# oss0430/SRFRD

Hardware: NVIDIA B200
Metric: training seqs/sec; full-catalogue top-10 users/sec (higher is better)
Workload: dtype bf16

## Files before the change

include/srfrd_b200.h:

```cpp
#ifndef SRFRD_B200_H
#define SRFRD_B200_H

#include <stddef.h>
#include <stdint.h>

#ifdef __cplusplus
extern "C" {
#endif

#define SRFRD_ABI_VERSION 9
#if defined(__GNUC__)
#define SRFRD_API __attribute__((visibility("default")))
#else
#define SRFRD_API
#endif

SRFRD_API const char* srfrd_last_error(void);
SRFRD_API int srfrd_abi_version(void);
SRFRD_API int srfrd_device_check(void);

SRFRD_API int srfrd_embed_ln_fwd(const float* item_table, int64_t n_rows, int D, const float* pos_table,
                       const float* aux_table, int64_t n_aux, int F, int mode, const int64_t* seq,
                       const int64_t* aux_ids, int64_t B, int L, float item_scale, const float* ln_w,
                       const float* ln_b, float eps, void* x0_bf16, float* x0_f32, void* q_bf16, float* stats,
                       int ldx, float drop_p, uint64_t drop_seed, uint32_t drop_stream, const float* drop_step,
                       void* stream);

SRFRD_API int srfrd_srfu_labels(const int64_t* fake_ids, int64_t B, int L, int kind, int64_t* labels, void* stream);

SRFRD_API int srfrd_embed_bwd(const void* dx0_bf16, int ldx, const int64_t* seq, const int64_t* aux_ids, int64_t B, int L,
                    int D, int F, int mode, float item_scale, float* d_item, float* d_aux, void* stream);

SRFRD_API int srfrd_layernorm_fwd(const void* x_bf16, int ldx, const float* w, const float* b, float eps, void* y_bf16,
                        float* y_f32, int ldy, float* stats, int64_t T, int H, int64_t row_stride,
                        int64_t row_offset, void* stream);
SRFRD_API int srfrd_layernorm_bwd(const void* dy_bf16, const float* dy_f32, int lddy, const void* x_bf16, int ldx,
                        const float* stats, const float* w, const void* add_bf16, int ldadd,
                        const int64_t* row_ids, void* dx_bf16, int lddx, float* dw, float* db, int64_t T, int H,
                        void* stream);

typedef struct {
  const float* bias;
  const void* residual;
  const void* gate;
  const int64_t* row_ids;
  void* out_bf16;
  float* out_f32;
  int ldr, ldg, ldc;
  int relu;
  float drop_p;
  uint32_t drop_stream;
  uint64_t drop_seed;
  const float* drop_step;
  void* ln_out_bf16;
  const float* ln_w;
  const float* ln_b;
  float* ln_stats;
  int ld_ln;
  float ln_eps;
} srfrd_gemm_epilogue_t;

SRFRD_API int srfrd_gemm_tn(const void* A_bf16, int lda, const void* B_bf16, int ldb, int M, int N, int K,
                  const srfrd_gemm_epilogue_t* ep, void* stream);
SRFRD_API int srfrd_gemm_tn_plan(int M, int N, int K, int has_aux, int bf16_out, int fused_ln, int* out);
SRFRD_API int srfrd_gemm_debug_read(long long* host_dst);
SRFRD_API int srfrd_attn_debug_read(long long* host_dst);

SRFRD_API int srfrd_gemm_wgrad(const void* dY_bf16, int lda, const void* X_bf16, int ldb, int64_t T, int Mo, int No,
                     float* dW, int ldw, float* dbias, void* stream);
SRFRD_API int srfrd_gemm_ref(const void* A, int lda, const void* B, int ldb, float* C, int ldc, int M, int N, int K,
                   int a_mn_major, int b_mn_major, void* stream);

SRFRD_API int srfrd_colsum(const void* X_bf16, int64_t M, int N, int64_t ld, float* out, void* stream);
SRFRD_API int srfrd_add_segments(float* in, int64_t n, int seg_in, int seg_out, float* out, void* stream);

SRFRD_API int srfrd_dropout_apply(const void* x_bf16, int ldx, void* out_bf16, int ldo, int64_t M, int N, float drop_p,
                        uint64_t seed, uint32_t stream_id, const float* drop_step, void* stream);

typedef struct {
  const float* src; int src_ld;
  void* dst; int dst_ld;
  void* dst_t; int dst_t_ld;
  int rows, cols;
  int dst_is_f32;
} srfrd_cast_desc_t;
SRFRD_API int srfrd_cast_weights(const srfrd_cast_desc_t* descs_dev, int n, void* stream);
SRFRD_API int srfrd_f32_to_bf16_split(const float* src, int64_t src_ld, const int64_t* row_index, void* hi, void* lo,
                            int64_t rows, int cols, int dst_ld, void* stream);

SRFRD_API int srfrd_attention_fwd(const void* q, int ldq, const void* k, const void* v, int ldkv, void* o, int ldo,
                        float* stats, int64_t B, int L, int H, int heads, float drop_p, uint64_t seed, uint32_t stream_id,
                        const float* drop_step, void* stream);
SRFRD_API int srfrd_attention_bwd(const void* dout, int lddo, const void* q, int ldq, const void* k, const void* v, int ldkv,
                        const void* o, int ldo, float* stats, void* dq, int lddq, void* dk, void* dv, int lddkv, int64_t B,
                        int L, int H, int heads, float drop_p, uint64_t seed, uint32_t stream_id, const float* drop_step,
                        void* stream);

SRFRD_API int srfrd_score_fwd(const float* h, int ldh, const float* item_table, const float* fake_table, const int64_t* pos,
                    const int64_t* neg, const int64_t* prs, const int64_t* nrs, int64_t T, int D, int F, float* zp,
                    float* zn, void* stream);
SRFRD_API int srfrd_score_bwd(const float* h, int ldh, const float* item_table, const float* fake_table, const int64_t* pos,
                    const int64_t* neg, const int64_t* prs, const int64_t* nrs, const float* dzp, const float* dzn,
                    int64_t T, int D, int F, float* dh, int lddh, float* d_item, float* d_fake, void* stream);
SRFRD_API int srfrd_score_loss_fused(const float* h, int ldh, const float* item_table, const float* fake_table,
                           const int64_t* pos, const int64_t* neg, const int64_t* prs, const int64_t* nrs,
                           const float* w_pos, const float* w_neg, const float* norm, int64_t T, int D, int F,
                           float* zp, float* zn, float* loss_acc, float* dh, int lddh, float* d_item, float* d_fake,
                           void* stream);
SRFRD_API int srfrd_weight_sums(const int64_t* pos, const float* w_pos, const float* w_neg, int64_t T, float* out2,
                      void* stream);
SRFRD_API int srfrd_loss_finalize(float* acc2, const float* norm2, float* loss, void* stream);

SRFRD_API int srfrd_adam_tick(float* state3, float beta1, float beta2, void* stream);
SRFRD_API int srfrd_adam_step(float* p, float* g, float* m, float* v, int64_t n, float lr, float beta1, float beta2, float eps,
                    const float* state3, int zero_grad, void* stream);

SRFRD_API int srfrd_adam_step_fused(float* p, float* g, float* m, float* v, int64_t n, float lr, float beta1, float beta2,
                          float eps, float* state8, int zero_grad, float* acc2, const float* norm2, float* loss,
                          void* stream, const int64_t* l2_seg, int l2_n_seg, const float* l2_coef, const float* l2_reg);

SRFRD_API int srfrd_param_l2_plan(const int64_t* seg_host, int n_seg, int64_t* n_chunks);
SRFRD_API int srfrd_param_l2(const float* p, const int64_t* seg, int n_seg, int64_t n_chunks, float l2, float* coef,
                   float* reg, double* ws, void* stream);

#define SRFRD_TOPK_KMAX 64
SRFRD_API int srfrd_catalogue_topk_plan(int64_t U, int64_t n_rows, int64_t row_lo, int D, int n_split, int* chunks_out,
                                        int k);
SRFRD_API int srfrd_catalogue_topk_kmax(int D, int n_split, int* kmax_out);
SRFRD_API int srfrd_catalogue_topk(const void* feats_bf16, int64_t U, int64_t u_pad, int n_split, const void* table_bf16,
                         int64_t n_rows, int64_t row_lo, int64_t id_base, int D, int ld_feats, int ld_table,
                         int chunks, float* part_scores, int* part_ids, float* packed_out, void* stream, int k);
SRFRD_API int srfrd_merge_topk(const float* scores, const int* ids, int64_t U, int nlists, int k, float* out_scores,
                     int64_t* out_ids, void* stream);
SRFRD_API int srfrd_merge_topk_packed(const float* packed, int64_t U, int nlists, int k, float* out_scores,
                            int64_t* out_ids, void* stream);
SRFRD_API int srfrd_catalogue_rank(const void* feats_bf16, int64_t U, int64_t u_pad, int n_split,
                                   const void* table_bf16, int64_t n_rows, int64_t row_lo, int64_t id_base,
                                   int D, int ld_feats, int ld_table,
                                   const void* target_rows_bf16, int ld_target, const int64_t* target_ids,
                                   float* target_scores, int* rank_out, void* stream);

SRFRD_API int srfrd_sample_batch(const int64_t* offsets, const int* items, const int8_t* labels, const float* p_fake,
                       const int* eligible, int n_eligible, int itemnum, int B, int L, int policy, uint64_t seed,
                       const float* step, int64_t* users, int64_t* seq, int64_t* rsq, int64_t* pos, int64_t* prs,
                       int64_t* neg, int64_t* nrs, float* w_pos, void* stream);

SRFRD_API int srfrd_sample_candidates(const int64_t* offsets, const int* items, const int* users0, const int* target,
                            int64_t U, int itemnum, int C, uint64_t seed, int64_t* cand, void* stream);
SRFRD_API int srfrd_candidate_rank(const float* feats, int ldf, const float* item_table, int64_t n_rows, int D,
                         const int64_t* cand, int64_t U, int C, const float* fake_table, int F,
                         const int64_t* user_label, float* logits, int ldl, int* rank, int* err_flag, void* stream);
SRFRD_API int srfrd_add_user_term(float* logits, int ldl, int64_t U, int I, const float* feats_tail, int ldf,
                        const float* fake_table, const int64_t* label, int F, void* stream);

typedef struct {
  int* rows;
  int* cnt;
  int* seq_first;
  int* tok_row;
  int* row_tok;
  int64_t* row_ids;
  int* row_info;
  int* tile_row0;
  int* last_row;
  int64_t cap;
} srfrd_pack_t;
SRFRD_API int srfrd_pack_plan(const int64_t* seq, const int64_t* keep, int64_t B, int L, const srfrd_pack_t* pk, void* stream);
SRFRD_API int srfrd_set_row_limit(const int* rows_dev);
SRFRD_API int srfrd_embed_ln_fwd_packed(const float* item_table, int64_t n_rows, int D, const float* pos_table,
                              const float* aux_table, int64_t n_aux, int F, int mode, const int64_t* seq,
                              const int64_t* aux_ids, int64_t B, int L, float item_scale, const float* ln_w,
                              const float* ln_b, float eps, void* x0_bf16, void* q_bf16, float* stats, int ldx,
                              float drop_p, uint64_t drop_seed, uint32_t drop_stream, const float* drop_step,
                              const int* row_tok, const int* rows_dev, int64_t cap_rows, void* stream);
SRFRD_API int srfrd_layernorm_fwd_rows(const void* x_bf16, int ldx, const float* w, const float* b, float eps, float* y_f32,
                             int ldy, const int* row_index, int64_t n, int H, void* stream);
SRFRD_API int srfrd_attention_packed_supported(int L, int H, int heads);
SRFRD_API int srfrd_attention_packed_oproj_supported(int L, int H, int heads);
SRFRD_API int srfrd_attention_fwd_packed(const void* q, int ldq, const void* k, const void* v, int ldkv, void* o, int ldo,
                               const srfrd_pack_t* pk, int L, int H, int heads, float drop_p, uint64_t seed,
                               uint32_t stream_id, const float* drop_step, void* stream, const void* wo, int ldw,
                               const float* bo, const void* res, int ldres, const float* ln_w, const float* ln_b,
                               float ln_eps, float* ln_stats, void* r, int ldr, void* y, int ldy);
SRFRD_API int srfrd_attention_bwd_packed(const void* dout, int lddo, const void* q, int ldq, const void* k, const void* v,
                               int ldkv, void* dq, int lddq, void* dk, void* dv, int lddkv, const srfrd_pack_t* pk,
                               int L, int H, int heads, float drop_p, uint64_t seed, uint32_t stream_id,
                               const float* drop_step, void* stream, const void* dr, int lddr, const void* woT, int ldw);
SRFRD_API int srfrd_score_loss_fused_packed(const float* h, int ldh, const float* item_table, const float* fake_table,
                                  const int64_t* pos, const int64_t* neg, const int64_t* prs, const int64_t* nrs,
                                  const float* w_pos, const float* w_neg, const float* norm, int D, int F,
                                  float* loss_acc, float* dh, int lddh, float* d_item, float* d_fake,
                                  const int* row_tok, const int* rows_dev, int64_t cap_rows, void* stream);
SRFRD_API int srfrd_embed_bwd_packed(const void* dx0_bf16, int ldx, const int64_t* seq, const int64_t* aux_ids,
                           const int* row_tok, const int* rows_dev, int64_t cap_rows, int L, int D, int F, int mode,
                           float item_scale, float* d_item, float* d_aux, float* d_pos, void* stream);

typedef struct {
  const float* bias1; const float* bias2;
  const void* gate; int ldg;
  int relu1;
  float drop1_p, drop2_p; uint32_t drop1_stream, drop2_stream; uint64_t drop_seed; const float* drop_step;
  const void* residual; int ldr;
  int residual_is_a;
  const int64_t* row_ids;
  void* mid_out; int ldm;
  void* out; int ldc;
  void* ln_out; int ld_ln; const float* ln_w; const float* ln_b; float* ln_stats; float ln_eps;
} srfrd_mlp2_t;
SRFRD_API int srfrd_mlp2_tn(const void* A_bf16, int lda, const void* W1_bf16, int ldw1, const void* W2_bf16, int ldw2, int M, int N,
                  const srfrd_mlp2_t* ep, void* stream);

SRFRD_API int srfrd_attention_live_items(const int* tok_row, int64_t B, int L, int heads, int* q_lo, int* items, int* n_live,
                               void* stream);
SRFRD_API int srfrd_set_attention_live(const int* q_lo, const int* items, const int* n_live, const int* tok_row);

typedef struct {
  const void* src; int ld_s;
  void* dst; int ld_d;
  int W;
  int mode;
} srfrd_repack_part_t;
SRFRD_API int srfrd_unpack_rows(const srfrd_repack_part_t* parts, int n_parts, const srfrd_pack_t* pk, int64_t B, int L,
                      void* stream);
SRFRD_API int srfrd_pack_rows(const srfrd_repack_part_t* parts, int n_parts, const srfrd_pack_t* pk, int64_t B, int L,
                    void* stream);

SRFRD_API int srfrd_dp_adam_step(float* const* grad_ptrs_dev, float* const* param_ptrs_dev, uint32_t* const* signal_ptrs_dev,
                       int rank, int world, int64_t n, float* m, float* v, float lr, float beta1, float beta2, float eps,
                       float* state8, const float* norm2, uint32_t* local4, void* stream, const int64_t* l2_seg,
                       int l2_n_seg, const float* l2_coef, const float* l2_reg);

#ifdef __cplusplus
}
#endif
#endif
```

srfrd_b200/_lib.py:

```python
from __future__ import annotations

import ctypes as C
import os

_HERE = os.path.dirname(os.path.abspath(__file__))
LIB_PATH = os.environ.get("SRFRD_B200_LIB") or os.path.join(_HERE, "lib", "libsrfrd_b200.so")

vp, i32, i64, f32, u32, u64 = C.c_void_p, C.c_int, C.c_int64, C.c_float, C.c_uint32, C.c_uint64


class GemmEpilogue(C.Structure):
    _fields_ = [("bias", vp), ("residual", vp), ("gate", vp), ("row_ids", vp), ("out_bf16", vp), ("out_f32", vp),
                ("ldr", i32), ("ldg", i32), ("ldc", i32), ("relu", i32), ("drop_p", f32), ("drop_stream", u32),
                ("drop_seed", u64), ("drop_step", vp),
                ("ln_out_bf16", vp), ("ln_w", vp), ("ln_b", vp), ("ln_stats", vp), ("ld_ln", i32), ("ln_eps", f32)]


class CastDesc(C.Structure):
    _fields_ = [("src", vp), ("src_ld", i32), ("dst", vp), ("dst_ld", i32), ("dst_t", vp), ("dst_t_ld", i32),
                ("rows", i32), ("cols", i32), ("dst_is_f32", i32)]


class Mlp2Epilogue(C.Structure):
    _fields_ = [("bias1", vp), ("bias2", vp), ("gate", vp), ("ldg", i32), ("relu1", i32), ("drop1_p", f32), ("drop2_p", f32),
                ("drop1_stream", u32), ("drop2_stream", u32), ("drop_seed", u64), ("drop_step", vp), ("residual", vp), ("ldr", i32),
                ("residual_is_a", i32), ("row_ids", vp), ("mid_out", vp), ("ldm", i32), ("out", vp), ("ldc", i32),
                ("ln_out", vp), ("ld_ln", i32), ("ln_w", vp), ("ln_b", vp), ("ln_stats", vp), ("ln_eps", f32)]


class PackDesc(C.Structure):
    _fields_ = [("rows", vp), ("cnt", vp), ("seq_first", vp), ("tok_row", vp), ("row_tok", vp), ("row_ids", vp),
                ("row_info", vp), ("tile_row0", vp), ("last_row", vp), ("cap", i64)]


class RepackPart(C.Structure):
    _fields_ = [("src", vp), ("ld_s", i32), ("dst", vp), ("ld_d", i32), ("W", i32), ("mode", i32)]


SIGNATURES = {
    "srfrd_abi_version": [],
    "srfrd_device_check": [],
    "srfrd_embed_ln_fwd": [vp, i64, i32, vp, vp, i64, i32, i32, vp, vp, i64, i32, f32, vp, vp, f32, vp, vp, vp, vp, i32,
                           f32, u64, u32, vp, vp],
    "srfrd_srfu_labels": [vp, i64, i32, i32, vp, vp],
    "srfrd_embed_bwd": [vp, i32, vp, vp, i64, i32, i32, i32, i32, f32, vp, vp, vp],
    "srfrd_layernorm_fwd": [vp, i32, vp, vp, f32, vp, vp, i32, vp, i64, i32, i64, i64, vp],
    "srfrd_layernorm_bwd": [vp, vp, i32, vp, i32, vp, vp, vp, i32, vp, vp, i32, vp, vp, i64, i32, vp],
    "srfrd_gemm_tn": [vp, i32, vp, i32, i32, i32, i32, C.POINTER(GemmEpilogue), vp],
    "srfrd_mlp2_tn": [vp, i32, vp, i32, vp, i32, i32, i32, C.POINTER(Mlp2Epilogue), vp],
    "srfrd_gemm_tn_plan": [i32, i32, i32, i32, i32, i32, vp],
    "srfrd_gemm_debug_read": [vp],
    "srfrd_attn_debug_read": [vp],
    "srfrd_gemm_wgrad": [vp, i32, vp, i32, i64, i32, i32, vp, i32, vp, vp],
    "srfrd_gemm_ref": [vp, i32, vp, i32, vp, i32, i32, i32, i32, i32, i32, vp],
    "srfrd_colsum": [vp, i64, i32, i64, vp, vp],
    "srfrd_add_segments": [vp, i64, i32, i32, vp, vp],
    "srfrd_dropout_apply": [vp, i32, vp, i32, i64, i32, f32, u64, u32, vp, vp],
    "srfrd_cast_weights": [vp, i32, vp],
    "srfrd_f32_to_bf16_split": [vp, i64, vp, vp, vp, i64, i32, i32, vp],
    "srfrd_attention_fwd": [vp, i32, vp, vp, i32, vp, i32, vp, i64, i32, i32, i32, f32, u64, u32, vp, vp],
    "srfrd_attention_bwd": [vp, i32, vp, i32, vp, vp, i32, vp, i32, vp, vp, i32, vp, vp, i32, i64, i32, i32, i32, f32, u64,
                            u32, vp, vp],
    "srfrd_score_fwd": [vp, i32, vp, vp, vp, vp, vp, vp, i64, i32, i32, vp, vp, vp],
    "srfrd_score_bwd": [vp, i32, vp, vp, vp, vp, vp, vp, vp, vp, i64, i32, i32, vp, i32, vp, vp, vp],
    "srfrd_score_loss_fused": [vp, i32, vp, vp, vp, vp, vp, vp, vp, vp, vp, i64, i32, i32, vp, vp, vp, vp, i32, vp, vp, vp],
    "srfrd_weight_sums": [vp, vp, vp, i64, vp, vp],
    "srfrd_loss_finalize": [vp, vp, vp, vp],
    "srfrd_adam_tick": [vp, f32, f32, vp],
    "srfrd_adam_step": [vp, vp, vp, vp, i64, f32, f32, f32, f32, vp, i32, vp],
    "srfrd_adam_step_fused": [vp, vp, vp, vp, i64, f32, f32, f32, f32, vp, i32, vp, vp, vp, vp, vp, i32, vp, vp],
    "srfrd_param_l2_plan": [C.POINTER(i64), i32, C.POINTER(i64)],
    "srfrd_param_l2": [vp, vp, i32, i64, f32, vp, vp, vp, vp],
    "srfrd_catalogue_topk_plan": [i64, i64, i64, i32, i32, C.POINTER(i32), i32],
    "srfrd_catalogue_topk_kmax": [i32, i32, C.POINTER(i32)],
    "srfrd_catalogue_topk": [vp, i64, i64, i32, vp, i64, i64, i64, i32, i32, i32, i32, vp, vp, vp, vp, i32],
    "srfrd_merge_topk_packed": [vp, i64, i32, i32, vp, vp, vp],
    "srfrd_catalogue_rank": [vp, i64, i64, i32, vp, i64, i64, i64, i32, i32, i32, vp, i32, vp, vp, vp, vp],
    "srfrd_attention_live_items": [vp, i64, i32, i32, vp, vp, vp, vp],
    "srfrd_set_attention_live": [vp, vp, vp, vp],
    "srfrd_merge_topk": [vp, vp, i64, i32, i32, vp, vp, vp],
    "srfrd_unpack_rows": [C.POINTER(RepackPart), i32, C.POINTER(PackDesc), i64, i32, vp],
    "srfrd_pack_rows": [C.POINTER(RepackPart), i32, C.POINTER(PackDesc), i64, i32, vp],
    "srfrd_dp_adam_step": [vp, vp, vp, i32, i32, i64, vp, vp, f32, f32, f32, f32, vp, vp, vp, vp, vp, i32, vp, vp],
    "srfrd_pack_plan": [vp, vp, i64, i32, C.POINTER(PackDesc), vp],
    "srfrd_set_row_limit": [vp],
    "srfrd_embed_ln_fwd_packed": [vp, i64, i32, vp, vp, i64, i32, i32, vp, vp, i64, i32, f32, vp, vp, f32, vp, vp, vp, i32,
                                  f32, u64, u32, vp, vp, vp, i64, vp],
    "srfrd_layernorm_fwd_rows": [vp, i32, vp, vp, f32, vp, i32, vp, i64, i32, vp],
    "srfrd_attention_packed_supported": [i32, i32, i32],
    "srfrd_attention_packed_oproj_supported": [i32, i32, i32],
    "srfrd_attention_fwd_packed": [vp, i32, vp, vp, i32, vp, i32, C.POINTER(PackDesc), i32, i32, i32, f32, u64, u32, vp, vp,
                                   vp, i32, vp, vp, i32, vp, vp, f32, vp, vp, i32, vp, i32],
    "srfrd_attention_bwd_packed": [vp, i32, vp, i32, vp, vp, i32, vp, i32, vp, vp, i32, C.POINTER(PackDesc), i32, i32, i32,
                                   f32, u64, u32, vp, vp, vp, i32, vp, i32],
    "srfrd_score_loss_fused_packed": [vp, i32, vp, vp, vp, vp, vp, vp, vp, vp, vp, i32, i32, vp, vp, i32, vp, vp, vp, vp,
                                      i64, vp],
    "srfrd_embed_bwd_packed": [vp, i32, vp, vp, vp, vp, i64, i32, i32, i32, i32, f32, vp, vp, vp, vp],
    "srfrd_sample_candidates": [vp, vp, vp, vp, i64, i32, i32, u64, vp, vp],
    "srfrd_candidate_rank": [vp, i32, vp, i64, i32, vp, i64, i32, vp, i32, vp, vp, i32, vp, vp, vp],
    "srfrd_add_user_term": [vp, i32, i64, i32, vp, i32, vp, vp, i32, vp],
    "srfrd_sample_batch": [vp, vp, vp, vp, vp, i32, i32, i32, i32, i32, u64, vp, vp, vp, vp, vp, vp, vp, vp, vp, vp],
}

_lib = None
_device_ok = False
launch_count = 0


def load() -> C.CDLL:
    global _lib
    if _lib is not None:
        return _lib
    if not os.path.exists(LIB_PATH):
        raise RuntimeError(
            f"srfrd_b200: {LIB_PATH} is not built. Run `make -C srfrd_b200/csrc` (needs nvcc, sm_100a). "
            "There is no CPU fallback.")
    lib = C.CDLL(LIB_PATH)
    lib.srfrd_last_error.restype = C.c_char_p
    lib.srfrd_last_error.argtypes = []
    for name, argtypes in SIGNATURES.items():
        fn = getattr(lib, name)
        fn.argtypes = argtypes
        fn.restype = C.c_int
    if lib.srfrd_abi_version() != 9:
        raise RuntimeError("srfrd_b200: ABI version mismatch between _lib.py and the built library")
    _lib = lib
    return lib


def require_device() -> None:
    global _device_ok
    if _device_ok:
        return
    lib = load()
    if lib.srfrd_device_check() != 0:
        raise RuntimeError("srfrd_b200: " + lib.srfrd_last_error().decode())
    _device_ok = True


_profile = None


def set_profile(records) -> None:
    global _profile
    _profile = records


def call(name: str, *args) -> None:
    global launch_count
    lib = _lib or load()
    if _profile is not None:
        import torch
        e0, e1 = torch.cuda.Event(enable_timing=True), torch.cuda.Event(enable_timing=True)
        e0.record()
        rc = getattr(lib, name)(*args)
        e1.record()
        _profile.append((name, args, e0, e1))
    else:
        rc = getattr(lib, name)(*args)
    if rc != 0:
        raise RuntimeError(f"{name}: {lib.srfrd_last_error().decode()}")
    launch_count += 1
```

srfrd_b200/csrc/ffn.cu:

```cuda
#include <stdlib.h>

#include "common.cuh"
#include "srfrd_b200.h"

namespace srfrd {

static constexpr int MLP_THREADS = 160;
static constexpr int MT = 128;
static constexpr int MBLK = MT * 64 * 2;

struct MlpParams {
  int M, N, kb;
  int K, kbk;
  int single;
  int relu2; const bf16* gate2; int ldg2;
  const int* rows_dev;
  const float *bias1, *bias2;
  const bf16* gate; int ldg;
  int relu1;
  uint64_t drop_seed; const float* drop_step;
  uint32_t thresh1, thresh2, stream1, stream2; float scale1, scale2;
  const bf16* residual; int ldr;
  int residual_is_a;
  const int64_t* row_ids;
  const float *ln_w, *ln_b; float* ln_stats; float ln_eps; int has_ln;
};

__device__ __forceinline__ uint32_t swz_chunk(int r, int j) { return (uint32_t)(r * 128 + ((j ^ (r & 7)) << 4)); }
__device__ __forceinline__ void mlp_bar_sync() { asm volatile("bar.sync 1, 128;" ::: "memory"); }
__device__ __forceinline__ void mlp_tma_store(const CUtensorMap* tmap, const void* smem_src, int c0, int c1) {
  asm volatile("cp.async.bulk.tensor.2d.global.shared::cta.bulk_group [%0, {%2, %3}], [%1];" ::"l"(tmap),
               "r"(smem_u32(smem_src)), "r"(c0), "r"(c1)
               : "memory");
}
__device__ __forceinline__ void unpack8_bf16(const uint4& u, float* f) {
  const uint32_t w[4] = {u.x, u.y, u.z, u.w};
#pragma unroll
  for (int i = 0; i < 4; ++i) { f[2 * i] = __uint_as_float(w[i] << 16); f[2 * i + 1] = __uint_as_float(w[i] & 0xffff0000u); }
}

__global__ void __launch_bounds__(MLP_THREADS, 2)
mlp2_kernel(const __grid_constant__ CUtensorMap tmA, const __grid_constant__ CUtensorMap tmW1,
            const __grid_constant__ CUtensorMap tmW2, const __grid_constant__ CUtensorMap tmMid,
            const __grid_constant__ CUtensorMap tmOut, const __grid_constant__ CUtensorMap tmLn, MlpParams p) {
  extern __shared__ uint8_t smem_raw[];
  uint8_t* smem = reinterpret_cast<uint8_t*>((reinterpret_cast<uintptr_t>(smem_raw) + 1023) & ~uintptr_t(1023));
  const int wblk = (p.N * 128 + 1023) & ~1023;
  const int ablk = max(p.kb, p.kbk);
  uint8_t* sW1 = smem;
  uint8_t* sW2 = sW1 + p.kbk * wblk;
  uint8_t* sA = sW2 + (p.single ? 0 : p.kb) * wblk;
  uint8_t* sM = sA + ablk * MBLK;
  float* sb1 = reinterpret_cast<float*>(sM + p.kb * MBLK);
  float* sb2 = sb1 + 128;
  float* slw = sb2 + 128;
  float* slb = slw + 128;
  uint64_t* bars = reinterpret_cast<uint64_t*>(slb + 128);
  uint64_t *w_full = bars, *a_full = bars + 1, *a_free = bars + 2, *acc1_full = bars + 3, *mid_ready = bars + 4,
           *acc2_full = bars + 5;
  uint32_t* tmem_slot = reinterpret_cast<uint32_t*>(bars + 6);
  const int warp = threadIdx.x >> 5, lane = threadIdx.x & 31;

  if (warp == 4 && lane == 0) {
    tma_prefetch_desc(&tmA); tma_prefetch_desc(&tmW1); tma_prefetch_desc(&tmW2); tma_prefetch_desc(&tmMid);
    tma_prefetch_desc(&tmOut);
    if (p.has_ln) tma_prefetch_desc(&tmLn);
    mbar_init(w_full, 1); mbar_init(a_full, 1); mbar_init(a_free, 1); mbar_init(acc1_full, 1); mbar_init(mid_ready, 1);
    mbar_init(acc2_full, 1);
    fence_barrier_init();
  }
  if (warp == 4) { tmem_alloc(tmem_slot, 256); tmem_relinquish(); }
  pdl_prologue_done();
  const int M = p.rows_dev ? min(p.M, __ldg(p.rows_dev)) : p.M;
  const int n_tiles = (M + MT - 1) / MT;
  for (int i = threadIdx.x; i < 128; i += blockDim.x) {
    sb1[i] = (p.bias1 && i < p.N) ? __ldg(p.bias1 + i) : 0.f;
    sb2[i] = (p.bias2 && i < p.N) ? __ldg(p.bias2 + i) : 0.f;
    slw[i] = (p.has_ln && i < p.N) ? __ldg(p.ln_w + i) : 0.f;
    slb[i] = (p.has_ln && i < p.N) ? __ldg(p.ln_b + i) : 0.f;
  }
  tc_fence_before();
  __syncthreads();
  tc_fence_after();
  const uint32_t tmem_base = *tmem_slot;
  const uint32_t tAcc1 = tmem_base, tAcc2 = tmem_base + 128;

  if (warp == 4) {
    if ((int)blockIdx.x < n_tiles && elect_one()) {
      mbar_expect_tx(w_full, (p.kbk + (p.single ? 0 : p.kb)) * p.N * 128);
      for (int kb = 0; kb < p.kbk; ++kb) tma_load_2d(sW1 + kb * wblk, &tmW1, w_full, kb * 64, 0, SRFRD_EVICT_LAST);
      if (!p.single)
        for (int kb = 0; kb < p.kb; ++kb) tma_load_2d(sW2 + kb * wblk, &tmW2, w_full, kb * 64, 0, SRFRD_EVICT_LAST);
    }
    __syncwarp();
    const uint32_t idesc = umma_idesc_bf16(MT, p.N, 0, 0);
    const uint64_t dA = umma_smem_desc(smem_u32(sA), 0, 1024), dM = umma_smem_desc(smem_u32(sM), 0, 1024);
    const uint64_t dW1 = umma_smem_desc(smem_u32(sW1), 0, 1024), dW2 = umma_smem_desc(smem_u32(sW2), 0, 1024);
    uint32_t ph = 0;
    for (int tile = blockIdx.x; tile < n_tiles; tile += gridDim.x, ph ^= 1) {
      mbar_wait(a_free, ph ^ 1);
      if (elect_one()) {
        mbar_expect_tx(a_full, p.kbk * MBLK);
        for (int kb = 0; kb < p.kbk; ++kb) tma_load_2d(sA + kb * MBLK, &tmA, a_full, kb * 64, tile * MT, SRFRD_EVICT_FIRST);
      }
      __syncwarp();
      if (tile == (int)blockIdx.x) mbar_wait(w_full, 0);
      mbar_wait(a_full, ph);
      tc_fence_after();
      if (elect_one()) {
        for (int kb = 0; kb < p.kbk; ++kb) {
          const int ksteps = min(4, (p.K - kb * 64 + 15) / 16);
          for (int k = 0; k < ksteps; ++k)
            umma_bf16(p.single ? tAcc2 : tAcc1, dA + (uint64_t)(kb * (MBLK >> 4) + 2 * k),
                      dW1 + (uint64_t)(kb * (wblk >> 4) + 2 * k), idesc, (kb | k) != 0);
        }
        umma_commit(p.single ? acc2_full : acc1_full);
      }
      __syncwarp();
      if (p.single) continue;
      mbar_wait(mid_ready, ph);
      tc_fence_after();
      if (elect_one()) {
        for (int kb = 0; kb < p.kb; ++kb) {
          const int ksteps = min(4, (p.N - kb * 64 + 15) / 16);
          for (int k = 0; k < ksteps; ++k)
            umma_bf16(tAcc2, dM + (uint64_t)(kb * (MBLK >> 4) + 2 * k), dW2 + (uint64_t)(kb * (wblk >> 4) + 2 * k), idesc, (kb | k) != 0);
        }
        umma_commit(acc2_full);
      }
      __syncwarp();
    }
  } else {
    const int r = warp * 32 + lane;
    const uint32_t lane_off = (uint32_t)(warp * 32) << 16;
    const uint64_t seed = (p.thresh1 | p.thresh2) ? mix_seed(p.drop_seed, p.drop_step) : 0;
    const bool issuer = threadIdx.x == 0;
    uint32_t ph = 0;
    for (int tile = blockIdx.x; tile < n_tiles; tile += gridDim.x, ph ^= 1) {
      const int64_t row = (int64_t)tile * MT + r;
      const bool rok = row < M;
      if (!p.single) {
      mbar_wait(acc1_full, ph);
      tc_fence_after();
#pragma unroll 1
      for (int c = 0; c < p.N; c += 16) {
        uint32_t raw[16];
        tmem_ld16(tAcc1 + lane_off + c, raw);
        uint4 g0 = make_uint4(0, 0, 0, 0), g1 = g0;
        if (p.gate && rok) {
          const uint4* gp = reinterpret_cast<const uint4*>(p.gate + row * p.ldg + c);
          g0 = __ldg(gp); g1 = __ldg(gp + 1);
        }
        tmem_ld_wait();
        float v[16], gv[16];
        if (p.gate) { unpack8_bf16(g0, gv); unpack8_bf16(g1, gv + 8); }
#pragma unroll
        for (int i = 0; i < 16; ++i) {
          float x = __uint_as_float(raw[i]) + sb1[c + i];
          if (p.thresh1)
            x = dropout_keep(seed, p.stream1, (uint64_t)row * (uint64_t)p.N + (uint64_t)(c + i), p.thresh1) ? x * p.scale1 : 0.f;
          if (p.relu1) x = fmaxf(x, 0.f);
          if (p.gate) x = gv[i] > 0.f ? x : 0.f;
          v[i] = x;
        }
        uint8_t* blk = sM + (c >> 6) * MBLK;
        const int j = (c & 63) >> 3;
        *reinterpret_cast<uint4*>(blk + swz_chunk(r, j)) =
            make_uint4(pack_bf16x2(v[0], v[1]), pack_bf16x2(v[2], v[3]), pack_bf16x2(v[4], v[5]), pack_bf16x2(v[6], v[7]));
        *reinterpret_cast<uint4*>(blk + swz_chunk(r, j + 1)) =
            make_uint4(pack_bf16x2(v[8], v[9]), pack_bf16x2(v[10], v[11]), pack_bf16x2(v[12], v[13]), pack_bf16x2(v[14], v[15]));
      }
      tc_fence_before();
      fence_proxy_async();
      mlp_bar_sync();
      if (issuer) {
        mbar_arrive(mid_ready);
        for (int kb = 0; kb < p.kb; ++kb) mlp_tma_store(&tmMid, sM + kb * MBLK, kb * 64, tile * MT);
        asm volatile("cp.async.bulk.commit_group;" ::: "memory");
      }
      }
      const float rowm = (p.row_ids && rok) ? ((__ldg(p.row_ids + row) != 0) ? 1.f : 0.f) : 1.f;
      mbar_wait(acc2_full, ph);
      tc_fence_after();
      float ln_sum = 0.f, ln_sq = 0.f;
#pragma unroll 1
      for (int c = 0; c < p.N; c += 16) {
        uint32_t raw[16];
        tmem_ld16(tAcc2 + lane_off + c, raw);
        uint8_t* blk = sA + (c >> 6) * MBLK;
        const int j = (c & 63) >> 3;
        uint4 r0 = make_uint4(0, 0, 0, 0), r1 = r0;
        if (p.residual_is_a && c < p.K) {
          r0 = *reinterpret_cast<const uint4*>(blk + swz_chunk(r, j));
          r1 = *reinterpret_cast<const uint4*>(blk + swz_chunk(r, j + 1));
        } else if (p.residual && rok) {
          const uint4* rp = reinterpret_cast<const uint4*>(p.residual + row * p.ldr + c);
          r0 = __ldg(rp); r1 = __ldg(rp + 1);
        }
        uint4 q0 = make_uint4(0, 0, 0, 0), q1 = q0;
        if (p.gate2 && rok) {
          const uint4* gp = reinterpret_cast<const uint4*>(p.gate2 + row * p.ldg2 + c);
          q0 = __ldg(gp); q1 = __ldg(gp + 1);
        }
        tmem_ld_wait();
        float v[16], rv[16], gv2[16];
        unpack8_bf16(r0, rv); unpack8_bf16(r1, rv + 8);
        if (p.gate2) { unpack8_bf16(q0, gv2); unpack8_bf16(q1, gv2 + 8); }
#pragma unroll
        for (int i = 0; i < 16; ++i) {
          float x = __uint_as_float(raw[i]) + sb2[c + i];
          if (p.thresh2)
            x = dropout_keep(seed, p.stream2, (uint64_t)row * (uint64_t)p.N + (uint64_t)(c + i), p.thresh2) ? x * p.scale2 : 0.f;
          if (p.relu2) x = fmaxf(x, 0.f);
          if (p.gate2) x = gv2[i] > 0.f ? x : 0.f;
          x += rv[i];
          v[i] = x * rowm;
        }
        const uint4 p0 = make_uint4(pack_bf16x2(v[0], v[1]), pack_bf16x2(v[2], v[3]), pack_bf16x2(v[4], v[5]), pack_bf16x2(v[6], v[7]));
        const uint4 p1 = make_uint4(pack_bf16x2(v[8], v[9]), pack_bf16x2(v[10], v[11]), pack_bf16x2(v[12], v[13]), pack_bf16x2(v[14], v[15]));
        *reinterpret_cast<uint4*>(blk + swz_chunk(r, j)) = p0;
        *reinterpret_cast<uint4*>(blk + swz_chunk(r, j + 1)) = p1;
        if (p.has_ln) {
          float q[16];
          unpack8_bf16(p0, q); unpack8_bf16(p1, q + 8);
#pragma unroll
          for (int i = 0; i < 16; ++i) { ln_sum += q[i]; ln_sq = fmaf(q[i], q[i], ln_sq); }
        }
      }
      tc_fence_before();
      if (p.has_ln) {
        if (issuer) asm volatile("cp.async.bulk.wait_group.read 0;" ::: "memory");
        mlp_bar_sync();
        const float invn = 1.f / (float)p.N;
        const float mean = ln_sum * invn;
        const float var = fmaxf(ln_sq * invn - mean * mean, 0.f);
        const float rstd = rsqrtf(var + p.ln_eps), nb = -mean * rstd;
#pragma unroll 1
        for (int c = 0; c < p.N; c += 8) {
          const int j = (c & 63) >> 3;
          const uint4 xv = *reinterpret_cast<const uint4*>(sA + (c >> 6) * MBLK + swz_chunk(r, j));
          float q[8], y[8];
          unpack8_bf16(xv, q);
#pragma unroll
          for (int i = 0; i < 8; ++i) y[i] = fmaf(fmaf(q[i], rstd, nb), slw[c + i], slb[c + i]);
          *reinterpret_cast<uint4*>(sM + (c >> 6) * MBLK + swz_chunk(r, j)) =
              make_uint4(pack_bf16x2(y[0], y[1]), pack_bf16x2(y[2], y[3]), pack_bf16x2(y[4], y[5]), pack_bf16x2(y[6], y[7]));
        }
        if (p.ln_stats && rok) *reinterpret_cast<float2*>(p.ln_stats + 2 * row) = make_float2(mean, rstd);
      }
      fence_proxy_async();
      mlp_bar_sync();
      if (issuer) {
        for (int kb = 0; kb < p.kb; ++kb) mlp_tma_store(&tmOut, sA + kb * MBLK, kb * 64, tile * MT);
        if (p.has_ln)
          for (int kb = 0; kb < p.kb; ++kb) mlp_tma_store(&tmLn, sM + kb * MBLK, kb * 64, tile * MT);
        asm volatile("cp.async.bulk.commit_group;" ::: "memory");
        asm volatile("cp.async.bulk.wait_group.read 0;" ::: "memory");
        mbar_arrive(a_free);
      }
    }
    if (issuer) asm volatile("cp.async.bulk.wait_group 0;" ::: "memory");
  }
  tc_fence_before();
  __syncthreads();
  if (warp == 4) { tc_fence_after(); tmem_dealloc(tmem_base, 256); }
}

}

using namespace srfrd;

static int mlp_launch(MlpParams& p, const void* A, int lda, const void* W1, int ldw1, const void* W2, int ldw2, void* mid_out,
                      int ldm, void* out, int ldc, void* ln_out, int ld_ln, cudaStream_t stream) {
  p.kb = (p.N + 63) / 64; p.kbk = (p.K + 63) / 64; p.rows_dev = row_limit();
  p.has_ln = ln_out != nullptr;
  CUtensorMap tmA, tmW1, tmW2, tmMid, tmOut, tmLn;
  if (int rc = make_tmap_bf16_2d(&tmA, A, p.M, p.K, lda, MT, 64)) return rc;
  if (int rc = make_tmap_bf16_2d(&tmW1, W1, p.N, p.K, ldw1, p.N, 64)) return rc;
  tmW2 = tmW1; tmMid = tmA;
  if (!p.single) {
    if (int rc = make_tmap_bf16_2d(&tmW2, W2, p.N, p.N, ldw2, p.N, 64)) return rc;
    if (int rc = make_tmap_bf16_2d(&tmMid, mid_out, p.M, p.N, ldm, MT, 64)) return rc;
  }
  if (int rc = make_tmap_bf16_2d(&tmOut, out, p.M, p.N, ldc, MT, 64)) return rc;
  tmLn = tmOut;
  if (p.has_ln) if (int rc = make_tmap_bf16_2d(&tmLn, ln_out, p.M, p.N, ld_ln, MT, 64)) return rc;
  const int wblk = (p.N * 128 + 1023) & ~1023;
  const int ablk = p.kb > p.kbk ? p.kb : p.kbk;
  const size_t smem = 1024 + (size_t)(p.kbk + (p.single ? 0 : p.kb)) * wblk + (size_t)(ablk + p.kb) * MBLK + 4 * 128 * sizeof(float) + 128;
  static bool attr = false;
  if (!attr) {
    SRFRD_CUDA(cudaFuncSetAttribute(mlp2_kernel, cudaFuncAttributeMaxDynamicSharedMemorySize, 200 * 1024));
    attr = true;
  }
  SRFRD_REQUIRE(smem <= 200 * 1024, "mlp2_tn: shared memory %zu too large", smem);
  int64_t grid = ((int64_t)p.M + MT - 1) / MT;
  if (grid > 2 * num_sms()) grid = 2 * num_sms();
  SRFRD_CUDA(launch_pdl(mlp2_kernel, dim3((unsigned)grid), dim3(MLP_THREADS), smem, stream, tmA, tmW1, tmW2, tmMid, tmOut, tmLn, p));
  SRFRD_LAUNCH_CHECK();
  return 0;
}

namespace srfrd {
bool gemm_small_eligible(int M, int N, int K, const srfrd_gemm_epilogue_t* ep, int lda, int ldb) {
  if (!ep->out_bf16 || ep->out_f32 || N > 128 || N % 16 || K > 128 || K % 8 || lda % 8 || ldb % 8 || ep->ldc % 8) return false;
  if (((uintptr_t)ep->out_bf16 & 15) || (ep->residual && (ep->ldr % 8 || ((uintptr_t)ep->residual & 15)))) return false;
  if (ep->gate && (ep->ldg % 8 || ((uintptr_t)ep->gate & 15))) return false;
  if (ep->residual && ep->gate) return false;
  if (ep->ln_out_bf16 && (!ep->ln_w || !ep->ln_b || ep->ld_ln % 8 || ((uintptr_t)ep->ln_out_bf16 & 15))) return false;
  { const char* e = getenv("SRFRD_LEAN_GEMM"); if (!e || e[0] != '1') return false; }
  return row_limit() != nullptr || M <= 32768;
}
int gemm_small_launch(const void* A, int lda, const void* B, int ldb, int M, int N, int K, const srfrd_gemm_epilogue_t* ep,
                      cudaStream_t stream) {
  MlpParams p = {};
  p.M = M; p.N = N; p.K = K; p.single = 1;
  p.bias2 = ep->bias; p.relu2 = ep->relu; p.gate2 = (const bf16*)ep->gate; p.ldg2 = ep->ldg;
  p.residual = (const bf16*)ep->residual; p.ldr = ep->ldr;
  p.residual_is_a = (ep->residual == A && ep->ldr == lda && N <= K) ? 1 : 0;
  if (p.residual_is_a) p.residual = nullptr;
  p.row_ids = ep->row_ids;
  p.drop_seed = ep->drop_seed; p.drop_step = ep->drop_step; p.stream2 = ep->drop_stream;
  p.thresh2 = ep->drop_p > 0.f ? (uint32_t)((double)ep->drop_p * 4294967296.0) : 0;
  p.scale2 = ep->drop_p > 0.f ? 1.f / (1.f - ep->drop_p) : 1.f;
  p.scale1 = 1.f;
  p.ln_w = ep->ln_w; p.ln_b = ep->ln_b; p.ln_stats = ep->ln_stats; p.ln_eps = ep->ln_eps;
  return mlp_launch(p, A, lda, B, ldb, nullptr, 0, nullptr, 0, ep->out_bf16, ep->ldc, ep->ln_out_bf16, ep->ld_ln, stream);
}
}

extern "C" int srfrd_mlp2_tn(const void* A, int lda, const void* W1, int ldw1, const void* W2, int ldw2, int M, int N,
                             const srfrd_mlp2_t* ep, void* stream_) {
  cudaStream_t stream = (cudaStream_t)stream_;
  SRFRD_REQUIRE(A && W1 && W2 && ep && ep->mid_out && ep->out, "mlp2_tn: null pointer");
  SRFRD_REQUIRE(M > 0 && N >= 16 && N <= 128 && N % 16 == 0, "mlp2_tn: N = K must be a multiple of 16 up to 128 (got %d)", N);
  SRFRD_REQUIRE(lda % 8 == 0 && ldw1 % 8 == 0 && ldw2 % 8 == 0 && ep->ldm % 8 == 0 && ep->ldc % 8 == 0 && lda >= N && ldw1 >= N &&
                    ldw2 >= N && ep->ldm >= N && ep->ldc >= N, "mlp2_tn: bad leading dimensions");
  SRFRD_REQUIRE(!ep->gate || (ep->ldg % 8 == 0 && ((uintptr_t)ep->gate & 15) == 0), "mlp2_tn: bad gate");
  SRFRD_REQUIRE(!ep->residual || (ep->ldr % 8 == 0 && ((uintptr_t)ep->residual & 15) == 0), "mlp2_tn: bad residual");
  SRFRD_REQUIRE(!ep->ln_out || (ep->ln_w && ep->ln_b && ep->ld_ln % 8 == 0 && ep->ld_ln >= N), "mlp2_tn: bad LayerNorm arguments");
  SRFRD_REQUIRE(ep->drop1_p >= 0.f && ep->drop1_p < 1.f && ep->drop2_p >= 0.f && ep->drop2_p < 1.f, "mlp2_tn: dropout p must be in [0, 1)");
  MlpParams p = {};
  p.M = M; p.N = N; p.K = N; p.single = 0;
  p.bias1 = ep->bias1; p.bias2 = ep->bias2; p.gate = (const bf16*)ep->gate; p.ldg = ep->ldg; p.relu1 = ep->relu1;
  p.drop_seed = ep->drop_seed; p.drop_step = ep->drop_step; p.stream1 = ep->drop1_stream; p.stream2 = ep->drop2_stream;
  p.thresh1 = ep->drop1_p > 0.f ? (uint32_t)((double)ep->drop1_p * 4294967296.0) : 0;
  p.thresh2 = ep->drop2_p > 0.f ? (uint32_t)((double)ep->drop2_p * 4294967296.0) : 0;
  p.scale1 = ep->drop1_p > 0.f ? 1.f / (1.f - ep->drop1_p) : 1.f;
  p.scale2 = ep->drop2_p > 0.f ? 1.f / (1.f - ep->drop2_p) : 1.f;
  p.residual = (const bf16*)ep->residual; p.ldr = ep->ldr;
  p.residual_is_a = (ep->residual == nullptr && ep->residual_is_a) || (ep->residual == A && ep->ldr == lda);
  if (p.residual_is_a) p.residual = nullptr;
  p.row_ids = ep->row_ids;
  p.ln_w = ep->ln_w; p.ln_b = ep->ln_b; p.ln_stats = ep->ln_stats; p.ln_eps = ep->ln_eps;
  return mlp_launch(p, A, lda, W1, ldw1, W2, ldw2, ep->mid_out, ep->ldm, ep->out, ep->ldc, ep->ln_out, ep->ld_ln, stream);
}
```

srfrd_b200/engine.py:

```python
from __future__ import annotations

import math
import os
from contextlib import contextmanager, nullcontext
from dataclasses import dataclass
from typing import Dict, List, Optional, Tuple

import torch

from . import ops

bf16 = torch.bfloat16
LN_EPS = 1e-8

KINDS = ("SRFR", "SRFRN", "SRFU_B", "SRFU_F", "SRFU_R", "SASRec")


@dataclass
class ModelSpec:
    kind: str
    item_number: int
    max_len: int
    D: int
    F: int = 0
    n_labels: int = 0
    num_blocks: int = 2
    num_heads: int = 1
    dropout: float = 0.0

    def __post_init__(self):
        if self.kind not in KINDS:
            raise ValueError(f"unknown model kind {self.kind}")
        if self.H % self.num_heads:
            raise ValueError("hidden size must be divisible by num_heads")
        if (self.H // self.num_heads) % 2:
            raise ValueError(f"srfrd_b200: head width {self.H // self.num_heads} must be even (bf16 pairs)")

    @property
    def H(self) -> int:
        return self.D + self.F if self.kind in ("SRFR", "SRFRN") else self.D

    @property
    def Dout(self) -> int:
        return self.H if self.kind == "SRFRN" else self.D

    @property
    def Hp(self) -> int:
        return (self.H + 15) // 16 * 16

    @property
    def Dp(self) -> int:
        return (self.D + 15) // 16 * 16

    @property
    def Doutp(self) -> int:
        return self.Hp if self.kind == "SRFRN" else self.Dp

    @property
    def padded(self) -> bool:
        return self.Hp != self.H or self.Dp != self.D

    @property
    def mode(self) -> int:
        return 1 if self.kind in ("SRFR", "SRFRN") else (2 if self.kind.startswith("SRFU") else 0)

    @property
    def item_scale(self) -> float:
        return float(self.D ** 0.5) if self.kind == "SASRec" else 1.0

    @property
    def item_key(self) -> str:
        return "item_emb.weight" if self.kind == "SASRec" else "embedding_layer.item_embed.weight"

    @property
    def pos_key(self) -> str:
        return "pos_emb.weight" if self.kind == "SASRec" else "embedding_layer.pos_embed.weight"

    @property
    def aux_key(self) -> Optional[str]:
        if self.mode == 1:
            return "embedding_layer.fake_embed.weight"
        if self.mode == 2:
            return "embedding_layer.user_label_embed.weight"
        return None

    def param_shapes(self) -> List[Tuple[str, Tuple[int, ...]]]:
        H, D, L, N = self.H, self.D, self.max_len, self.item_number
        out: List[Tuple[str, Tuple[int, ...]]] = []
        if self.kind == "SASRec":
            out += [("item_emb.weight", (N + 1, D)), ("pos_emb.weight", (L, D))]
        elif self.mode == 1:
            out += [("embedding_layer.item_embed.weight", (N + 1, D)),
                    ("embedding_layer.fake_embed.weight", (3, self.F)),
                    ("embedding_layer.pos_embed.weight", (L, D))]
        else:
            out += [("embedding_layer.item_embed.weight", (N + 1, D)),
                    ("embedding_layer.user_label_embed.weight", (self.n_labels, D)),
                    ("embedding_layer.pos_embed.weight", (L, D))]
        for i in range(self.num_blocks):
            out += [(f"attention_layernorms.{i}.weight", (H,)), (f"attention_layernorms.{i}.bias", (H,))]
        for i in range(self.num_blocks):
            out += [(f"attention_layers.{i}.in_proj_weight", (3 * H, H)), (f"attention_layers.{i}.in_proj_bias", (3 * H,)),
                    (f"attention_layers.{i}.out_proj.weight", (H, H)), (f"attention_layers.{i}.out_proj.bias", (H,))]
        for i in range(self.num_blocks):
            out += [(f"forward_layernorms.{i}.weight", (H,)), (f"forward_layernorms.{i}.bias", (H,))]
        for i in range(self.num_blocks):
            out += [(f"forward_layers.{i}.conv1.weight", (H, H, 1)), (f"forward_layers.{i}.conv1.bias", (H,)),
                    (f"forward_layers.{i}.conv2.weight", (H, H, 1)), (f"forward_layers.{i}.conv2.bias", (H,))]
        if self.kind == "SRFR":
            out += [("last_conv.weight", (D, H, 1)), ("last_conv.bias", (D,))]
        out += [("last_layernorm.weight", (self.Dout,)), ("last_layernorm.bias", (self.Dout,))]
        return out


class FlatParams:

    def __init__(self, spec: ModelSpec, device, alloc=None):
        self.spec = spec
        self.offsets: Dict[str, Tuple[int, Tuple[int, ...]]] = {}
        off = 0
        for name, shape in spec.param_shapes():
            n = int(math.prod(shape))
            self.offsets[name] = (off, shape)
            off += (n + 3) // 4 * 4
        self.numel = off
        zeros = (lambda n: alloc(n).zero_()) if alloc is not None else (lambda n: torch.zeros(n, dtype=torch.float32, device=device))
        self.data_ext = zeros(off + 4)
        self.data = self.data_ext[:off]
        self.data_tail = self.data_ext[off:]
        self.grad_bucket = zeros(off + 4)
        self.grad = self.grad_bucket[:off]
        self.grad_tail = self.grad_bucket[off:]

    def segments(self) -> List[Tuple[int, int]]:
        return [(off, int(math.prod(shape))) for off, shape in self.offsets.values()]

    def view(self, name: str, grad: bool = False) -> torch.Tensor:
        off, shape = self.offsets[name]
        buf = self.grad if grad else self.data
        return buf[off:off + int(math.prod(shape))].view(shape)

    def mat(self, name: str, grad: bool = False) -> torch.Tensor:
        v = self.view(name, grad)
        return v.view(v.shape[0], -1)


class HotPath:

    def __init__(self, spec: ModelSpec, params: FlatParams):
        self.spec, self.P = spec, params
        self.device = params.data.device
        self._ws_tokens = 0
        self._ws: Dict[str, torch.Tensor] = {}
        self.ws_generation = 0
        self.fwd_version = 0
        self.host_drop_counter = 0
        self._build_shadows()
        self.step_state = torch.zeros(8, dtype=torch.float32, device=self.device)
        self.side = torch.cuda.Stream(device=self.device)
        self.side2 = torch.cuda.Stream(device=self.device)
        self.overlap = os.environ.get("SRFRD_OVERLAP", "1") != "0"
        self.drop_seed = 0x5EED5EED
        self.saved: Optional[dict] = None
        self._plans: Dict[Tuple[int, int], ops.PackedPlan] = {}
        self.packed_default = os.environ.get("SRFRD_PACKED", "1") != "0"
        self.fuse_ffn = os.environ.get("SRFRD_FUSE_FFN", "1") != "0"

    def _build_shadows(self):
        s, P, dev = self.spec, self.P, self.device
        H, D, Hp, Dp = s.H, s.D, s.Hp, s.Dp
        self.sh: Dict[str, torch.Tensor] = {}
        self.vsh: Dict[str, torch.Tensor] = {}
        entries = []
        zb = lambda r, c: torch.zeros(r, c, dtype=bf16, device=dev)

        def vec(name, src, n_pad, dst_off=0, dst=None):
            if not s.padded:
                return
            if dst is None:
                dst = self.vsh.setdefault(name, torch.zeros(n_pad, dtype=torch.float32, device=dev))
            entries.append((src.view(1, -1), dst[dst_off:dst_off + src.numel()].view(1, -1), None))

        for i in range(s.num_blocks):
            win = P.mat(f"attention_layers.{i}.in_proj_weight")
            bin_ = P.view(f"attention_layers.{i}.in_proj_bias")
            self.sh[f"wq{i}"] = zb(Hp, Hp)
            self.sh[f"wkv{i}"] = zb(2 * Hp, Hp)
            self.sh[f"wqT{i}"] = zb(Hp, Hp)
            self.sh[f"wkvT{i}"] = zb(Hp, 2 * Hp)
            entries.append((win[:H], self.sh[f"wq{i}"][:H, :H], self.sh[f"wqT{i}"][:H, :H]))
            entries.append((win[H:2 * H], self.sh[f"wkv{i}"][:H, :H], self.sh[f"wkvT{i}"][:H, :H]))
            entries.append((win[2 * H:], self.sh[f"wkv{i}"][Hp:Hp + H, :H], self.sh[f"wkvT{i}"][:H, Hp:Hp + H]))
            vec(f"bq{i}", bin_[:H], Hp)
            vec(f"bkv{i}", bin_[H:2 * H], 2 * Hp)
            vec(f"bkv{i}", bin_[2 * H:], 2 * Hp, dst_off=Hp)
            for tag, key in (("wo", f"attention_layers.{i}.out_proj"), ("w1", f"forward_layers.{i}.conv1"),
                             ("w2", f"forward_layers.{i}.conv2")):
                self.sh[f"{tag}{i}"] = zb(Hp, Hp)
                self.sh[f"{tag}T{i}"] = zb(Hp, Hp)
                entries.append((P.mat(key + ".weight"), self.sh[f"{tag}{i}"][:H, :H], self.sh[f"{tag}T{i}"][:H, :H]))
                vec(f"b{tag[1]}{i}", P.view(key + ".bias"), Hp)
        if s.kind == "SRFR":
            self.sh["wc"] = zb(Dp, Hp)
            self.sh["wcT"] = zb(Hp, Dp)
            entries.append((P.mat("last_conv.weight"), self.sh["wc"][:D, :H], self.sh["wcT"][:H, :D]))
            vec("bc", P.view("last_conv.bias"), Dp)
        self._cast_table, self._cast_n = ops.make_cast_table(entries, dev)
        self.shadows_version = -1

    def bias(self, tag: str, i: Optional[int] = None) -> torch.Tensor:
        s, P = self.spec, self.P
        if s.padded:
            return self.vsh[tag if i is None else f"{tag}{i}"]
        if tag == "bq":
            return P.view(f"attention_layers.{i}.in_proj_bias")[:s.H]
        if tag == "bkv":
            return P.view(f"attention_layers.{i}.in_proj_bias")[s.H:]
        if tag == "bc":
            return P.view("last_conv.bias")
        key = {"bo": f"attention_layers.{i}.out_proj.bias", "b1": f"forward_layers.{i}.conv1.bias",
               "b2": f"forward_layers.{i}.conv2.bias"}[tag]
        return P.view(key)

    def refresh_shadows(self):
        ops.cast_weights(self._cast_table, self._cast_n)

    @contextmanager
    def _branch(self, second: bool = False):
        if not self.overlap:
            yield
            return
        main = torch.cuda.current_stream()
        st = self.side2 if second else self.side
        st.wait_stream(main)
        with torch.cuda.stream(st):
            yield

    def _join(self, second: bool = False):
        if self.overlap:
            torch.cuda.current_stream().wait_stream(self.side2 if second else self.side)

    def _workspace(self, T: int, L: int) -> Dict[str, torch.Tensor]:
        if T <= self._ws_tokens:
            return self._ws
        s, dev = self.spec, self.device
        Lmax = max(L, s.max_len)
        H, nb = s.Hp, s.num_blocks
        ws: Dict[str, torch.Tensor] = {}

        def act(name, w=H, dtype=bf16):
            ws[name] = torch.zeros(T, w, dtype=dtype, device=dev)

        for i in range(nb + 1):
            act(f"x{i}")
        for i in range(nb):
            for n in ("Q", "q", "o", "r", "y", "h1"):
                act(f"{n}{i}")
            act(f"kv{i}", 2 * H)
            act(f"st1_{i}", 2, torch.float32)
            act(f"st2_{i}", 2, torch.float32)
            if Lmax > 128:
                ws[f"ast{i}"] = torch.zeros(T * s.num_heads, 4, dtype=torch.float32, device=dev)
        if s.kind == "SRFR":
            act("c", s.Dp)
        act("stF", 2, torch.float32)
        act("hfin", s.Doutp, torch.float32)
        act("dh", s.Doutp, torch.float32)
        for n in ("gA", "gC", "gD", "gX"):
            act(n)
        for i in range(nb):
            for n in ("gda1_", "gdr_", "gdq_"):
                act(f"{n}{i}")
            act(f"gdz_{i}")
            act(f"gdkv_{i}", 2 * H)
        if s.kind == "SRFR":
            act("gc", s.Dp)
        if s.dropout > 0:
            for i in range(nb):
                act(f"gE_{i}")
        ws["pos_tmp"] = torch.zeros(Lmax * H, dtype=torch.float32, device=dev)
        self._ws, self._ws_tokens = ws, T
        self.ws_generation += 1
        return ws

    def packed_ok(self, B: int, L: int) -> bool:
        return self.packed_mode(B, L) is not None

    def packed_mode(self, B: int, L: int) -> Optional[str]:
        s = self.spec
        if s.padded or s.H % 16 or s.D % 8 or B > 16384 or B < 1:
            return None
        if ops.attention_packed_supported(L, s.H, s.num_heads):
            return "tile"
        if os.environ.get("SRFRD_HYBRID", "1") != "0" and L <= 4096:
            return "hybrid"
        return None

    def _hybrid_ws(self, Td: int) -> Dict[str, torch.Tensor]:
        hw = getattr(self, "_hws", None)
        if hw is not None and hw["_rows"] >= Td:
            return hw
        s, dev = self.spec, self.device
        Hp = s.Hp
        hw = {"_rows": Td}
        z = lambda w: torch.zeros(Td, w, dtype=bf16, device=dev)
        for i in range(s.num_blocks):
            hw[f"qd{i}"], hw[f"kvd{i}"], hw[f"od{i}"] = z(Hp), z(2 * Hp), z(Hp)
        hw["dod"], hw["dqd"], hw["dkvd"] = z(Hp), z(Hp), z(2 * Hp)
        self._hws = hw
        self.ws_generation += 1
        return hw

    def _live_tiles(self, B: int, L: int) -> "ops.LiveTiles":
        key = (B, L)
        lt = getattr(self, "_lives", None)
        if lt is None:
            lt = self._lives = {}
        if key not in lt:
            if len(lt) >= 4:
                lt.clear()
                self.ws_generation += 1
            lt[key] = ops.LiveTiles(B, L, self.spec.num_heads, self.device)
        return lt[key]

    def _plan(self, B: int, L: int) -> "ops.PackedPlan":
        key = (B, L)
        if key not in self._plans:
            if len(self._plans) >= 4:
                self._plans.clear()
                self.ws_generation += 1
            self._plans[key] = ops.PackedPlan(B, L, self.device)
        return self._plans[key]

    def forward(self, seq: torch.Tensor, fake_ids: Optional[torch.Tensor], training: bool,
                last_only: bool = False, save: Optional[bool] = None, packed: bool = False,
                keep: Optional[torch.Tensor] = None) -> torch.Tensor:
        s, P = self.spec, self.P
        B, L = seq.shape
        if L > s.max_len:
            raise RuntimeError(f"sequence length {L} exceeds max_len {s.max_len} (pos_embed rows, SRFR_model.py:12)")
        if packed:
            return self._forward_packed(seq, fake_ids, training, last_only, save, keep)
        T, H, Hp, nb = B * L, s.H, s.Hp, s.num_blocks
        ws = self._workspace(T, L)
        self.fwd_version += 1
        p_drop = s.dropout if training else 0.0
        step = self.step_state[3:4] if p_drop > 0 else None
        seed = (self.drop_seed + self.host_drop_counter * 0x9E3779B97F4A7C15) & 0xFFFFFFFFFFFFFFFF
        seq = seq.contiguous()
        aux_ids = None
        if s.mode == 1:
            aux_ids = None if fake_ids is None else fake_ids.contiguous()
        elif s.mode == 2:
            aux_ids = torch.empty(B, dtype=torch.int64, device=self.device)
            ops.srfu_labels(fake_ids.contiguous(), {"SRFU_B": 0, "SRFU_F": 1, "SRFU_R": 2}[s.kind], aux_ids)
            need = {"SRFU_B": 3, "SRFU_F": L + 1, "SRFU_R": 11}[s.kind]
            if s.n_labels < need and B > 0 and int(aux_ids.max()) >= s.n_labels:
                raise IndexError(f"index out of range in self: {s.kind} user label {int(aux_ids.max())} needs "
                                 f"number_of_labels >= {need}, got {s.n_labels}")
        aux_table = P.view(s.aux_key) if s.aux_key else None
        x = [ws[f"x{i}"][:T] for i in range(nb + 1)]
        ops.embed_ln_fwd(P.view(s.item_key), P.view(s.pos_key), aux_table, s.mode, seq, aux_ids, s.item_scale,
                         P.view("attention_layernorms.0.weight"), P.view("attention_layernorms.0.bias"), LN_EPS,
                         x0_bf16=x[0], q_bf16=ws["Q0"][:T], stats=ws["st1_0"][:T],
                         drop_p=p_drop if s.kind == "SASRec" else 0.0, drop_seed=seed, drop_stream=1, drop_step=step)
        seq_flat = seq.view(-1)
        fuse_ln = (H == Hp) and Hp <= 128 and os.environ.get("SRFRD_FUSE_LN", "1") != "0"
        for i in range(nb):
            Q, q, kv, o, r, y, h1 = (ws[f"{n}{i}"][:T] for n in ("Q", "q", "kv", "o", "r", "y", "h1"))
            with self._branch():
                ops.gemm_tn(x[i], self.sh[f"wkv{i}"], out_bf16=kv, bias=self.bias("bkv", i))
            if i > 0 and not fuse_ln:
                ops.layernorm_fwd(x[i], P.view(f"attention_layernorms.{i}.weight"), P.view(f"attention_layernorms.{i}.bias"),
                                  LN_EPS, y_bf16=Q, stats=ws[f"st1_{i}"][:T], H=H)
            ops.gemm_tn(Q, self.sh[f"wq{i}"], out_bf16=q, bias=self.bias("bq", i))
            self._join()
            ops.attention_fwd(q, kv[:, :Hp], kv[:, Hp:], o, B, L, H, s.num_heads, p_drop, seed, 10 + 4 * i, step,
                              stats=ws.get(f"ast{i}"))
            if fuse_ln:
                ops.gemm_tn(o, self.sh[f"wo{i}"], out_bf16=r, bias=self.bias("bo", i), residual=Q, ln_out=y,
                            ln_w=P.view(f"forward_layernorms.{i}.weight"), ln_b=P.view(f"forward_layernorms.{i}.bias"),
                            ln_eps=LN_EPS, ln_stats=ws[f"st2_{i}"][:T])
            else:
                ops.gemm_tn(o, self.sh[f"wo{i}"], out_bf16=r, bias=self.bias("bo", i), residual=Q)
                ops.layernorm_fwd(r, P.view(f"forward_layernorms.{i}.weight"), P.view(f"forward_layernorms.{i}.bias"), LN_EPS,
                                  y_bf16=y, stats=ws[f"st2_{i}"][:T], H=H)
            ops.gemm_tn(y, self.sh[f"w1{i}"], out_bf16=h1, bias=self.bias("b1", i), relu=True,
                        drop_p=p_drop, drop_seed=seed, drop_stream=11 + 4 * i, drop_step=step)
            nxt = {}
            if fuse_ln and i + 1 < nb:
                nxt = dict(ln_out=ws[f"Q{i + 1}"][:T], ln_w=P.view(f"attention_layernorms.{i + 1}.weight"),
                           ln_b=P.view(f"attention_layernorms.{i + 1}.bias"), ln_eps=LN_EPS, ln_stats=ws[f"st1_{i + 1}"][:T])
            ops.gemm_tn(h1, self.sh[f"w2{i}"], out_bf16=x[i + 1], bias=self.bias("b2", i),
                        residual=y, row_ids=seq_flat, drop_p=p_drop, drop_seed=seed, drop_stream=12 + 4 * i, drop_step=step,
                        **nxt)
        fin_in = x[nb]
        if s.kind == "SRFR":
            ops.gemm_tn(x[nb], self.sh["wc"], out_bf16=ws["c"][:T], bias=self.bias("bc"))
            fin_in = ws["c"][:T]
        hfin = ws["hfin"][:T]
        if last_only:
            out = ws["hfin"][:B]
            ops.layernorm_fwd(fin_in, P.view("last_layernorm.weight"), P.view("last_layernorm.bias"), LN_EPS, y_f32=out,
                              T=B, H=s.Dout, row_stride=L, row_offset=L - 1)
            return out[:, :s.Dout]
        ops.layernorm_fwd(fin_in, P.view("last_layernorm.weight"), P.view("last_layernorm.bias"), LN_EPS, y_f32=hfin,
                          stats=ws["stF"][:T], H=s.Dout)
        if training if save is None else save:
            self.saved = dict(seq=seq, aux_ids=aux_ids, B=B, L=L, p_drop=p_drop, seed=seed, step=step,
                              version=self.fwd_version)
        return hfin.view(B, L, s.Doutp)[..., :s.Dout]

    def backward(self, dh: torch.Tensor, version: Optional[int] = None) -> None:
        s, P, sv = self.spec, self.P, self.saved
        if sv is None:
            raise RuntimeError("backward() without a training forward()")
        if sv["version"] != self.fwd_version or (version is not None and version != sv["version"]):
            raise RuntimeError("srfrd_b200: backward() of a stale forward -- another forward() (training, validation or "
                               "predict) ran on this model after the one being back-propagated and overwrote the shared "
                               "activation workspace; run backward() before the next forward()")
        if sv.get("plan") is not None:
            return self._backward_packed(dh)
        B, L = sv["B"], sv["L"]
        T, H, Hp, nb = B * L, s.H, s.Hp, s.num_blocks
        ws = self._ws
        seq_flat = sv["seq"].view(-1)
        p_drop, seed, step = sv["p_drop"], sv["seed"], sv["step"]
        gA, gC, gD, gX = (ws[n][:T] for n in ("gA", "gC", "gD", "gX"))
        G = lambda name: P.view(name, grad=True)
        GM = lambda name: P.mat(name, grad=True)
        x = [ws[f"x{i}"][:T] for i in range(nb + 1)]
        dz_top = ws[f"gdz_{nb - 1}"][:T]

        if s.kind == "SRFR":
            gc = ws["gc"][:T]
            ops.layernorm_bwd(dh, ws["c"][:T], ws["stF"][:T], P.view("last_layernorm.weight"), gc,
                              G("last_layernorm.weight"), G("last_layernorm.bias"), H=s.D)
            with self._branch():
                ops.gemm_wgrad(gc, x[nb], GM("last_conv.weight"), G("last_conv.bias"), Mo=s.D, No=H)
            ops.gemm_tn(gc, self.sh["wcT"], out_bf16=dz_top, row_ids=seq_flat)
        else:
            ops.layernorm_bwd(dh, x[nb], ws["stF"][:T], P.view("last_layernorm.weight"), dz_top,
                              G("last_layernorm.weight"), G("last_layernorm.bias"), row_ids=seq_flat, H=s.Dout)

        for i in reversed(range(nb)):
            Q, q, kv, o, r, y, h1 = (ws[f"{n}{i}"][:T] for n in ("Q", "q", "kv", "o", "r", "y", "h1"))
            dz, da1, dr, dq, dkv = (ws[f"{n}{i}"][:T] for n in ("gdz_", "gda1_", "gdr_", "gdq_", "gdkv_"))
            dx_out = ws[f"gdz_{i - 1}"][:T] if i > 0 else gA
            dz2 = dz
            if p_drop > 0:
                dz2 = ws[f"gE_{i}"][:T]
                ops.dropout_apply(dz, dz2, Hp, p_drop, seed, 12 + 4 * i, step)
            with self._branch():
                ops.gemm_wgrad(dz2, h1, GM(f"forward_layers.{i}.conv2.weight"), G(f"forward_layers.{i}.conv2.bias"), Mo=H, No=H)
            ops.gemm_tn(dz2, self.sh[f"w2T{i}"], out_bf16=da1, gate=h1, drop_p=p_drop, drop_seed=seed,
                        drop_stream=11 + 4 * i, drop_step=step)
            with self._branch():
                ops.gemm_wgrad(da1, y, GM(f"forward_layers.{i}.conv1.weight"), G(f"forward_layers.{i}.conv1.bias"), Mo=H, No=H)
            ops.gemm_tn(da1, self.sh[f"w1T{i}"], out_bf16=gC, residual=dz)
            ops.layernorm_bwd(gC, r, ws[f"st2_{i}"][:T], P.view(f"forward_layernorms.{i}.weight"), dr,
                              G(f"forward_layernorms.{i}.weight"), G(f"forward_layernorms.{i}.bias"), H=H)
            with self._branch():
                ops.gemm_wgrad(dr, o, GM(f"attention_layers.{i}.out_proj.weight"), G(f"attention_layers.{i}.out_proj.bias"),
                               Mo=H, No=H)
            ops.gemm_tn(dr, self.sh[f"woT{i}"], out_bf16=gC)
            ops.attention_bwd(gC, q, kv[:, :Hp], kv[:, Hp:], dq, dkv[:, :Hp], dkv[:, Hp:], B, L, H, s.num_heads, p_drop,
                              seed, 10 + 4 * i, step, o=o, stats=ws.get(f"ast{i}"))
            gin = GM(f"attention_layers.{i}.in_proj_weight")
            gbin = G(f"attention_layers.{i}.in_proj_bias")
            with self._branch():
                ops.gemm_wgrad(dq, Q, gin[:H], gbin[:H], Mo=H, No=H)
                if Hp == H:
                    ops.gemm_wgrad(dkv, x[i], gin[H:], gbin[H:], Mo=2 * H, No=H)
                else:
                    ops.gemm_wgrad(dkv[:, :Hp], x[i], gin[H:2 * H], gbin[H:2 * H], Mo=H, No=H)
                    ops.gemm_wgrad(dkv[:, Hp:], x[i], gin[2 * H:], gbin[2 * H:], Mo=H, No=H)
            with self._branch(second=True):
                ops.gemm_tn(dkv, self.sh[f"wkvT{i}"], out_bf16=gX)
            ops.gemm_tn(dq, self.sh[f"wqT{i}"], out_bf16=gD, residual=dr)
            self._join(second=True)
            ops.layernorm_bwd(gD, x[i], ws[f"st1_{i}"][:T], P.view(f"attention_layernorms.{i}.weight"), dx_out,
                              G(f"attention_layernorms.{i}.weight"), G(f"attention_layernorms.{i}.bias"),
                              add=gX, row_ids=seq_flat, H=H)

        dx0 = gA
        if s.kind == "SASRec" and p_drop > 0:
            ops.dropout_apply(gA, gC, H, p_drop, seed, 1, step)
            dx0 = gC
        aux_grad = G(s.aux_key) if s.aux_key else None
        ops.embed_bwd(dx0, sv["seq"], sv["aux_ids"], s.D, s.F if s.mode == 1 else 0, s.mode, s.item_scale,
                      G(s.item_key), aux_grad)
        pos_tmp = ws["pos_tmp"][:L * Hp]
        ops.colsum(dx0, pos_tmp, M=B, N=L * Hp, ld=L * Hp)
        ops.add_segments(pos_tmp, L * Hp, Hp, s.D, G(s.pos_key))
        self._join()
        self.saved = None

    def _forward_packed(self, seq, fake_ids, training, last_only, save, keep):
        s, P = self.spec, self.P
        B, L = seq.shape
        H, Hp, nb = s.H, s.Hp, s.num_blocks
        plan = self._plan(B, L)
        T = plan.cap
        ws = self._workspace(T, L)
        self.fwd_version += 1
        p_drop = s.dropout if training else 0.0
        step = self.step_state[3:4] if p_drop > 0 else None
        seed = (self.drop_seed + self.host_drop_counter * 0x9E3779B97F4A7C15) & 0xFFFFFFFFFFFFFFFF
        seq = seq.contiguous()
        aux_ids = None
        if s.mode == 1:
            aux_ids = None if fake_ids is None else fake_ids.contiguous()
        elif s.mode == 2:
            aux_ids = torch.empty(B, dtype=torch.int64, device=self.device)
            ops.srfu_labels(fake_ids.contiguous(), {"SRFU_B": 0, "SRFU_F": 1, "SRFU_R": 2}[s.kind], aux_ids)
            need = {"SRFU_B": 3, "SRFU_F": L + 1, "SRFU_R": 11}[s.kind]
            if s.n_labels < need and int(aux_ids.max()) >= s.n_labels:
                raise IndexError(f"index out of range in self: {s.kind} user label {int(aux_ids.max())} needs "
                                 f"number_of_labels >= {need}, got {s.n_labels}")
        aux_table = P.view(s.aux_key) if s.aux_key else None
        plan.build(seq, None if keep is None else keep.contiguous())
        hyb = self._hybrid_ws(B * L) if self.packed_mode(B, L) == "hybrid" else None
        live = None
        if hyb is not None and os.environ.get("SRFRD_LIVE_TILES", "1") != "0":
            live = self._live_tiles(B, L)
            live.build(plan)
        x = [ws[f"x{i}"][:T] for i in range(nb + 1)]
        row_ids = plan.row_ids
        fuse_ln = Hp <= 128 and os.environ.get("SRFRD_FUSE_LN", "1") != "0"
        fuse_oproj = self._fuse_oproj(hyb, L, fuse_ln) & 1
        with ops.row_limit(plan.rows):
            ops.embed_ln_fwd_packed(P.view(s.item_key), P.view(s.pos_key), aux_table, s.mode, seq, aux_ids, s.item_scale,
                                    P.view("attention_layernorms.0.weight"), P.view("attention_layernorms.0.bias"), LN_EPS,
                                    x[0], ws["Q0"][:T], ws["st1_0"][:T], plan,
                                    drop_p=p_drop if s.kind == "SASRec" else 0.0, drop_seed=seed, drop_stream=1, drop_step=step)
            for i in range(nb):
                Q, q, kv, o, r, y, h1 = (ws[f"{n}{i}"][:T] for n in ("Q", "q", "kv", "o", "r", "y", "h1"))
                with self._branch():
                    ops.gemm_tn(x[i], self.sh[f"wkv{i}"], out_bf16=kv, bias=self.bias("bkv", i))
                if i > 0 and not fuse_ln:
                    ops.layernorm_fwd(x[i], P.view(f"attention_layernorms.{i}.weight"), P.view(f"attention_layernorms.{i}.bias"),
                                      LN_EPS, y_bf16=Q, stats=ws[f"st1_{i}"][:T], H=H)
                ops.gemm_tn(Q, self.sh[f"wq{i}"], out_bf16=q, bias=self.bias("bq", i))
                self._join()
                if fuse_oproj:
                    ops.attention_fwd_packed(q, kv[:, :Hp], kv[:, Hp:], o, plan, L, H, s.num_heads, p_drop, seed, 10 + 4 * i, step,
                                             wo=self.sh[f"wo{i}"], bias=self.bias("bo", i), residual=Q, r=r, y=y,
                                             ln_w=P.view(f"forward_layernorms.{i}.weight"),
                                             ln_b=P.view(f"forward_layernorms.{i}.bias"), ln_eps=LN_EPS,
                                             ln_stats=ws[f"st2_{i}"][:T])
                elif hyb is None:
                    ops.attention_fwd_packed(q, kv[:, :Hp], kv[:, Hp:], o, plan, L, H, s.num_heads, p_drop, seed, 10 + 4 * i, step)
                else:
                    qd, kvd, od = hyb[f"qd{i}"][:B * L], hyb[f"kvd{i}"][:B * L], hyb[f"od{i}"][:B * L]
                    ops.unpack_rows([(q, qd, Hp, 0), (kv, kvd, 2 * Hp, 0)], plan)
                    with (live.active() if live is not None else nullcontext()):
                        ops.attention_fwd(qd, kvd[:, :Hp], kvd[:, Hp:], od, B, L, H, s.num_heads, p_drop, seed, 10 + 4 * i, step,
                                          stats=ws.get(f"ast{i}"))
                    ops.pack_rows([(od, o, Hp, 0)], plan)
                if fuse_oproj:
                    pass
                elif fuse_ln:
                    ops.gemm_tn(o, self.sh[f"wo{i}"], out_bf16=r, bias=self.bias("bo", i), residual=Q, ln_out=y,
                                ln_w=P.view(f"forward_layernorms.{i}.weight"), ln_b=P.view(f"forward_layernorms.{i}.bias"),
                                ln_eps=LN_EPS, ln_stats=ws[f"st2_{i}"][:T])
                else:
                    ops.gemm_tn(o, self.sh[f"wo{i}"], out_bf16=r, bias=self.bias("bo", i), residual=Q)
                    ops.layernorm_fwd(r, P.view(f"forward_layernorms.{i}.weight"), P.view(f"forward_layernorms.{i}.bias"),
                                      LN_EPS, y_bf16=y, stats=ws[f"st2_{i}"][:T], H=H)
                nxt = {}
                if fuse_ln and i + 1 < nb:
                    nxt = dict(ln_out=ws[f"Q{i + 1}"][:T], ln_w=P.view(f"attention_layernorms.{i + 1}.weight"),
                               ln_b=P.view(f"attention_layernorms.{i + 1}.bias"), ln_eps=LN_EPS,
                               ln_stats=ws[f"st1_{i + 1}"][:T])
                if self.fuse_ffn and Hp <= 128:
                    ops.mlp2_tn(y, self.sh[f"w1{i}"], self.sh[f"w2{i}"], h1, x[i + 1], bias1=self.bias("b1", i),
                                bias2=self.bias("b2", i), relu1=True, drop1_p=p_drop, drop2_p=p_drop, drop1_stream=11 + 4 * i,
                                drop2_stream=12 + 4 * i, drop_seed=seed, drop_step=step, residual_is_a=True, row_ids=row_ids,
                                **nxt)
                else:
                    ops.gemm_tn(y, self.sh[f"w1{i}"], out_bf16=h1, bias=self.bias("b1", i), relu=True,
                                drop_p=p_drop, drop_seed=seed, drop_stream=11 + 4 * i, drop_step=step)
                    ops.gemm_tn(h1, self.sh[f"w2{i}"], out_bf16=x[i + 1], bias=self.bias("b2", i), residual=y, row_ids=row_ids,
                                drop_p=p_drop, drop_seed=seed, drop_stream=12 + 4 * i, drop_step=step, **nxt)
            fin_in = x[nb]
            if s.kind == "SRFR":
                ops.gemm_tn(x[nb], self.sh["wc"], out_bf16=ws["c"][:T], bias=self.bias("bc"))
                fin_in = ws["c"][:T]
            if not last_only:
                ops.layernorm_fwd(fin_in, P.view("last_layernorm.weight"), P.view("last_layernorm.bias"), LN_EPS,
                                  y_f32=ws["hfin"][:T], stats=ws["stF"][:T], H=s.Dout)
        if last_only:
            out = ws["hfin"][:B]
            ops.layernorm_fwd_rows(fin_in, P.view("last_layernorm.weight"), P.view("last_layernorm.bias"), LN_EPS, out,
                                   plan.last_row, B, s.Dout)
            return out[:, :s.Dout]
        if training if save is None else save:
            self.saved = dict(seq=seq, aux_ids=aux_ids, B=B, L=L, p_drop=p_drop, seed=seed, step=step,
                              version=self.fwd_version, plan=plan, hyb=hyb, live=live)
        return ws["hfin"][:T]

    def _fuse_oproj(self, hyb, L, fuse_ln) -> int:
        s = self.spec
        if hyb is not None or s.num_heads != 1 or not fuse_ln or s.Hp != s.H:
            return 0
        return ops.attention_packed_oproj_supported(L, s.H, s.num_heads)

    def _backward_packed(self, dh: torch.Tensor) -> None:
        s, P, sv = self.spec, self.P, self.saved
        plan, hyb, live = sv["plan"], sv.get("hyb"), sv.get("live")
        B, L = sv["B"], sv["L"]
        T, H, Hp, nb = plan.cap, s.H, s.Hp, s.num_blocks
        ws = self._ws
        row_ids = plan.row_ids
        p_drop, seed, step = sv["p_drop"], sv["seed"], sv["step"]
        gA, gC, gD, gX = (ws[n][:T] for n in ("gA", "gC", "gD", "gX"))
        G = lambda name: P.view(name, grad=True)
        GM = lambda name: P.mat(name, grad=True)
        x = [ws[f"x{i}"][:T] for i in range(nb + 1)]
        dz_top = ws[f"gdz_{nb - 1}"][:T]
        fuse_oproj = self._fuse_oproj(hyb, L, Hp <= 128 and os.environ.get("SRFRD_FUSE_LN", "1") != "0") & 2
        with ops.row_limit(plan.rows):
            if s.kind == "SRFR":
                gc = ws["gc"][:T]
                ops.layernorm_bwd(dh, ws["c"][:T], ws["stF"][:T], P.view("last_layernorm.weight"), gc,
                                  G("last_layernorm.weight"), G("last_layernorm.bias"), H=s.D)
                with self._branch():
                    ops.gemm_wgrad(gc, x[nb], GM("last_conv.weight"), G("last_conv.bias"), Mo=s.D, No=H)
                ops.gemm_tn(gc, self.sh["wcT"], out_bf16=dz_top, row_ids=row_ids)
            else:
                ops.layernorm_bwd(dh, x[nb], ws["stF"][:T], P.view("last_layernorm.weight"), dz_top,
                                  G("last_layernorm.weight"), G("last_layernorm.bias"), row_ids=row_ids, H=s.Dout)
            for i in reversed(range(nb)):
                Q, q, kv, o, r, y, h1 = (ws[f"{n}{i}"][:T] for n in ("Q", "q", "kv", "o", "r", "y", "h1"))
                dz, da1, dr, dq, dkv = (ws[f"{n}{i}"][:T] for n in ("gdz_", "gda1_", "gdr_", "gdq_", "gdkv_"))
                dx_out = ws[f"gdz_{i - 1}"][:T] if i > 0 else gA
                dz2 = dz
                if p_drop > 0:
                    dz2 = ws[f"gE_{i}"][:T]
                    ops.dropout_apply(dz, dz2, Hp, p_drop, seed, 12 + 4 * i, step)
                with self._branch():
                    ops.gemm_wgrad(dz2, h1, GM(f"forward_layers.{i}.conv2.weight"), G(f"forward_layers.{i}.conv2.bias"), Mo=H, No=H)
                if self.fuse_ffn and Hp <= 128:
                    ops.mlp2_tn(dz2, self.sh[f"w2T{i}"], self.sh[f"w1T{i}"], da1, gC, gate=h1, drop1_p=p_drop,
                                drop1_stream=11 + 4 * i, drop_seed=seed, drop_step=step, residual=dz)
                    with self._branch():
                        ops.gemm_wgrad(da1, y, GM(f"forward_layers.{i}.conv1.weight"), G(f"forward_layers.{i}.conv1.bias"),
                                       Mo=H, No=H)
                else:
                    ops.gemm_tn(dz2, self.sh[f"w2T{i}"], out_bf16=da1, gate=h1, drop_p=p_drop, drop_seed=seed,
                                drop_stream=11 + 4 * i, drop_step=step)
                    with self._branch():
                        ops.gemm_wgrad(da1, y, GM(f"forward_layers.{i}.conv1.weight"), G(f"forward_layers.{i}.conv1.bias"),
                                       Mo=H, No=H)
                    ops.gemm_tn(da1, self.sh[f"w1T{i}"], out_bf16=gC, residual=dz)
                ops.layernorm_bwd(gC, r, ws[f"st2_{i}"][:T], P.view(f"forward_layernorms.{i}.weight"), dr,
                                  G(f"forward_layernorms.{i}.weight"), G(f"forward_layernorms.{i}.bias"), H=H)
                with self._branch():
                    ops.gemm_wgrad(dr, o, GM(f"attention_layers.{i}.out_proj.weight"),
                                   G(f"attention_layers.{i}.out_proj.bias"), Mo=H, No=H)
                if not fuse_oproj:
                    ops.gemm_tn(dr, self.sh[f"woT{i}"], out_bf16=gC)
                if fuse_oproj:
                    ops.attention_bwd_packed(None, q, kv[:, :Hp], kv[:, Hp:], dq, dkv[:, :Hp], dkv[:, Hp:], plan, L, H,
                                             s.num_heads, p_drop, seed, 10 + 4 * i, step, dr=dr, woT=self.sh[f"woT{i}"])
                elif hyb is None:
                    ops.attention_bwd_packed(gC, q, kv[:, :Hp], kv[:, Hp:], dq, dkv[:, :Hp], dkv[:, Hp:], plan, L, H,
                                             s.num_heads, p_drop, seed, 10 + 4 * i, step)
                else:
                    Td = B * L
                    qd, kvd, od = hyb[f"qd{i}"][:Td], hyb[f"kvd{i}"][:Td], hyb[f"od{i}"][:Td]
                    dod, dqd, dkvd = hyb["dod"][:Td], hyb["dqd"][:Td], hyb["dkvd"][:Td]
                    ops.unpack_rows([(gC, dod, Hp, 1)], plan)
                    with (live.active() if live is not None else nullcontext()):
                        ops.attention_bwd(dod, qd, kvd[:, :Hp], kvd[:, Hp:], dqd, dkvd[:, :Hp], dkvd[:, Hp:], B, L, H,
                                          s.num_heads, p_drop, seed, 10 + 4 * i, step, o=od, stats=ws.get(f"ast{i}"))
                    ops.pack_rows([(dqd, dq, Hp, 0), (dkvd, dkv, 2 * Hp, 1)], plan)
                gin = GM(f"attention_layers.{i}.in_proj_weight")
                gbin = G(f"attention_layers.{i}.in_proj_bias")
                with self._branch():
                    ops.gemm_wgrad(dq, Q, gin[:H], gbin[:H], Mo=H, No=H)
                    ops.gemm_wgrad(dkv, x[i], gin[H:], gbin[H:], Mo=2 * H, No=H)
                with self._branch(second=True):
                    ops.gemm_tn(dkv, self.sh[f"wkvT{i}"], out_bf16=gX)
                ops.gemm_tn(dq, self.sh[f"wqT{i}"], out_bf16=gD, residual=dr)
                self._join(second=True)
                ops.layernorm_bwd(gD, x[i], ws[f"st1_{i}"][:T], P.view(f"attention_layernorms.{i}.weight"), dx_out,
                                  G(f"attention_layernorms.{i}.weight"), G(f"attention_layernorms.{i}.bias"),
                                  add=gX, row_ids=row_ids, H=H)
            dx0 = gA
            if s.kind == "SASRec" and p_drop > 0:
                ops.dropout_apply(gA, gC, H, p_drop, seed, 1, step)
                dx0 = gC
        aux_grad = G(s.aux_key) if s.aux_key else None
        ops.embed_bwd_packed(dx0, sv["seq"], sv["aux_ids"], plan, s.D, s.F if s.mode == 1 else 0, s.mode, s.item_scale,
                             G(s.item_key), aux_grad, G(s.pos_key))
        self._join()
        self.saved = None

    def fake_table(self) -> Optional[torch.Tensor]:
        return self.P.view("embedding_layer.fake_embed.weight") if self.spec.kind == "SRFRN" else None

    def fake_table_grad(self) -> Optional[torch.Tensor]:
        return self.P.view("embedding_layer.fake_embed.weight", grad=True) if self.spec.kind == "SRFRN" else None
```

srfrd_b200/ops.py:

```python
from __future__ import annotations

import ctypes as C
from typing import Optional

import torch

from . import _lib
from contextlib import contextmanager

from ._lib import CastDesc, GemmEpilogue, Mlp2Epilogue, PackDesc, RepackPart, call

bf16 = torch.bfloat16


def _p(t: Optional[torch.Tensor]):
    return None if t is None else t.data_ptr()


def _stream():
    return torch.cuda.current_stream().cuda_stream


def _chk(t: torch.Tensor, dtype, name: str):
    if not t.is_cuda:
        raise RuntimeError(f"srfrd_b200: {name} must be a CUDA tensor (there is no CPU fallback)")
    if t.dtype != dtype:
        raise RuntimeError(f"srfrd_b200: {name} must be {dtype}, got {t.dtype}")
    if t.stride(-1) != 1:
        raise RuntimeError(f"srfrd_b200: {name} must be contiguous in its last dimension")


def embed_ln_fwd(item_table, pos_table, aux_table, mode, seq, aux_ids, item_scale, ln_w, ln_b, eps,
                 x0_bf16=None, x0_f32=None, q_bf16=None, stats=None, drop_p=0.0, drop_seed=0, drop_stream=0,
                 drop_step=None):
    _lib.require_device()
    B, L = seq.shape
    D = item_table.shape[1]
    F = aux_table.shape[1] if (aux_table is not None and mode == 1) else 0
    _chk(item_table, torch.float32, "item_table"); _chk(seq, torch.int64, "seq")
    ldx = (x0_bf16 if x0_bf16 is not None else q_bf16).stride(0) if (x0_bf16 is not None or q_bf16 is not None) else D + F
    call("srfrd_embed_ln_fwd", _p(item_table), item_table.shape[0], D, _p(pos_table), _p(aux_table),
         0 if aux_table is None else aux_table.shape[0], F, mode, _p(seq), _p(aux_ids), B, L, float(item_scale),
         _p(ln_w), _p(ln_b), float(eps), _p(x0_bf16), _p(x0_f32), _p(q_bf16), _p(stats), ldx, float(drop_p),
         int(drop_seed), int(drop_stream), _p(drop_step), _stream())


def srfu_labels(fake_ids, kind: int, labels):
    _lib.require_device()
    B, L = fake_ids.shape
    call("srfrd_srfu_labels", _p(fake_ids), B, L, kind, _p(labels), _stream())


def embed_bwd(dx0, seq, aux_ids, D, F, mode, item_scale, d_item, d_aux):
    B, L = seq.shape
    call("srfrd_embed_bwd", _p(dx0), dx0.stride(0), _p(seq), _p(aux_ids), B, L, D, F, mode, float(item_scale),
         _p(d_item), _p(d_aux), _stream())


def layernorm_fwd(x, w, b, eps, y_bf16=None, y_f32=None, stats=None, T=None, H=None, row_stride=1, row_offset=0):
    _lib.require_device()
    T = x.shape[0] if T is None else T
    H = x.shape[1] if H is None else H
    y = y_bf16 if y_bf16 is not None else y_f32
    call("srfrd_layernorm_fwd", _p(x), x.stride(0), _p(w), _p(b), float(eps), _p(y_bf16), _p(y_f32), y.stride(0),
         _p(stats), T, H, row_stride, row_offset, _stream())


def layernorm_bwd(dy, x, stats, w, dx, dw, db, add=None, row_ids=None, H=None):
    T = x.shape[0]
    H = x.shape[1] if H is None else H
    dyb = dy if dy.dtype == bf16 else None
    dyf = dy if dy.dtype == torch.float32 else None
    call("srfrd_layernorm_bwd", _p(dyb), _p(dyf), dy.stride(0), _p(x), x.stride(0), _p(stats), _p(w), _p(add),
         0 if add is None else add.stride(0), _p(row_ids), _p(dx), dx.stride(0), _p(dw), _p(db), T, H, _stream())


def gemm_tn(A, B, out_bf16=None, out_f32=None, bias=None, residual=None, gate=None, row_ids=None, relu=False,
            drop_p=0.0, drop_seed=0, drop_stream=0, drop_step=None, M=None, ln_out=None, ln_w=None, ln_b=None, ln_eps=0.0,
            ln_stats=None):
    _lib.require_device()
    M = A.shape[0] if M is None else M
    K = A.shape[1]
    N = B.shape[0]
    out = out_bf16 if out_bf16 is not None else out_f32
    ep = GemmEpilogue(_p(bias), _p(residual), _p(gate), _p(row_ids), _p(out_bf16), _p(out_f32),
                      0 if residual is None else residual.stride(0), 0 if gate is None else gate.stride(0),
                      out.stride(0), int(relu), float(drop_p), int(drop_stream), int(drop_seed), _p(drop_step),
                      _p(ln_out), _p(ln_w), _p(ln_b), _p(ln_stats), 0 if ln_out is None else ln_out.stride(0), float(ln_eps))
    call("srfrd_gemm_tn", _p(A), A.stride(0), _p(B), B.stride(0), M, N, K, C.byref(ep), _stream())


def gemm_wgrad(dY, X, dW, dbias=None, Mo=None, No=None):
    T = dY.shape[0]
    Mo = dY.shape[1] if Mo is None else Mo
    No = X.shape[1] if No is None else No
    call("srfrd_gemm_wgrad", _p(dY), dY.stride(0), _p(X), X.stride(0), T, Mo, No, _p(dW), dW.stride(0), _p(dbias),
         _stream())


def gemm_ref(A, B, Cout, a_mn_major=False, b_mn_major=False):
    _lib.require_device()
    M, N = Cout.shape
    K = A.shape[0] if a_mn_major else A.shape[1]
    call("srfrd_gemm_ref", _p(A), A.stride(0), _p(B), B.stride(0), _p(Cout), Cout.stride(0), M, N, K,
         int(a_mn_major), int(b_mn_major), _stream())


def colsum(X, out, M=None, N=None, ld=None):
    M = X.shape[0] if M is None else M
    N = X.shape[1] if N is None else N
    ld = X.stride(0) if ld is None else ld
    call("srfrd_colsum", _p(X), M, N, ld, _p(out), _stream())


def add_segments(src, n, seg_in, seg_out, out):
    call("srfrd_add_segments", _p(src), n, seg_in, seg_out, _p(out), _stream())


def dropout_apply(x, out, N, drop_p, seed, stream_id, drop_step=None):
    call("srfrd_dropout_apply", _p(x), x.stride(0), _p(out), out.stride(0), x.shape[0], N, float(drop_p), int(seed),
         int(stream_id), _p(drop_step), _stream())


def cast_weights(descs_dev, n):
    call("srfrd_cast_weights", _p(descs_dev), n, _stream())


def make_cast_table(entries, device):
    arr = (CastDesc * len(entries))()
    for i, (src, dst, dst_t) in enumerate(entries):
        is_f32 = int(dst is not None and dst.dtype == torch.float32)
        arr[i] = CastDesc(src.data_ptr(), src.stride(0), _p(dst), 0 if dst is None else dst.stride(0), _p(dst_t),
                          0 if dst_t is None else dst_t.stride(0), src.shape[0], src.shape[1], is_f32)
    raw = bytes(arr)
    host = torch.frombuffer(bytearray(raw), dtype=torch.uint8)
    return host.to(device), len(entries)


def f32_to_bf16_split(src, hi, lo=None, row_index=None):
    _lib.require_device()
    rows = src.shape[0] if row_index is None else row_index.numel()
    cols = src.shape[1]
    call("srfrd_f32_to_bf16_split", _p(src), src.stride(0), _p(row_index), _p(hi), _p(lo), rows, cols, hi.stride(0),
         _stream())


def attention_fwd(q, k, v, o, B, L, H, heads, drop_p=0.0, seed=0, stream_id=0, drop_step=None, stats=None):
    _lib.require_device()
    call("srfrd_attention_fwd", _p(q), q.stride(0), _p(k), _p(v), k.stride(0), _p(o), o.stride(0), _p(stats), B, L, H, heads,
         float(drop_p), int(seed), int(stream_id), _p(drop_step), _stream())


def attention_bwd(dout, q, k, v, dq, dk, dv, B, L, H, heads, drop_p=0.0, seed=0, stream_id=0, drop_step=None, o=None,
                  stats=None):
    call("srfrd_attention_bwd", _p(dout), dout.stride(0), _p(q), q.stride(0), _p(k), _p(v), k.stride(0), _p(o),
         0 if o is None else o.stride(0), _p(stats), _p(dq), dq.stride(0), _p(dk), _p(dv), dk.stride(0), B, L, H, heads,
         float(drop_p), int(seed), int(stream_id), _p(drop_step), _stream())


def score_fwd(h, item_table, fake_table, pos, neg, prs, nrs, zp, zn):
    _lib.require_device()
    T = pos.numel()
    D = item_table.shape[1]
    F = 0 if fake_table is None else fake_table.shape[1]
    call("srfrd_score_fwd", _p(h), h.stride(0), _p(item_table), _p(fake_table), _p(pos), _p(neg), _p(prs), _p(nrs), T,
         D, F, _p(zp), _p(zn), _stream())


def score_bwd(h, item_table, fake_table, pos, neg, prs, nrs, dzp, dzn, dh, d_item, d_fake):
    T = pos.numel()
    D = item_table.shape[1]
    F = 0 if fake_table is None else fake_table.shape[1]
    call("srfrd_score_bwd", _p(h), h.stride(0), _p(item_table), _p(fake_table), _p(pos), _p(neg), _p(prs), _p(nrs),
         _p(dzp), _p(dzn), T, D, F, _p(dh), dh.stride(0), _p(d_item), _p(d_fake), _stream())


def score_loss_fused(h, item_table, fake_table, pos, neg, prs, nrs, w_pos, w_neg, norm, loss_acc, dh, d_item, d_fake,
                     zp=None, zn=None):
    T = pos.numel()
    D = item_table.shape[1]
    F = 0 if fake_table is None else fake_table.shape[1]
    call("srfrd_score_loss_fused", _p(h), h.stride(0), _p(item_table), _p(fake_table), _p(pos), _p(neg), _p(prs),
         _p(nrs), _p(w_pos), _p(w_neg), _p(norm), T, D, F, _p(zp), _p(zn), _p(loss_acc), _p(dh),
         0 if dh is None else dh.stride(0), _p(d_item), _p(d_fake), _stream())


def weight_sums(pos, w_pos, w_neg, out2):
    _lib.require_device()
    call("srfrd_weight_sums", _p(pos), _p(w_pos), _p(w_neg), pos.numel(), _p(out2), _stream())


def loss_finalize(acc2, norm2, loss):
    call("srfrd_loss_finalize", _p(acc2), _p(norm2), _p(loss), _stream())


def adam_tick(state3, beta1, beta2):
    call("srfrd_adam_tick", _p(state3), float(beta1), float(beta2), _stream())


def adam_step(p, g, m, v, lr, beta1, beta2, eps, state3, zero_grad=True):
    _lib.require_device()
    call("srfrd_adam_step", _p(p), _p(g), _p(m), _p(v), p.numel(), float(lr), float(beta1), float(beta2), float(eps),
         _p(state3), int(zero_grad), _stream())


def adam_step_fused(p, g, m, v, lr, beta1, beta2, eps, state8, zero_grad=True, acc2=None, norm2=None, loss=None,
                    l2: Optional["ParamL2"] = None):
    _lib.require_device()
    call("srfrd_adam_step_fused", _p(p), _p(g), _p(m), _p(v), p.numel(), float(lr), float(beta1), float(beta2), float(eps),
         _p(state8), int(zero_grad), _p(acc2), _p(norm2), _p(loss), _stream(), *_l2_args(l2))


class ParamL2:

    def __init__(self, segments, l2: float, device):
        host = (C.c_int64 * (2 * len(segments)))(*[int(x) for s in segments for x in s])
        n_chunks = C.c_int64(0)
        call("srfrd_param_l2_plan", host, len(segments), C.byref(n_chunks))
        self.n_seg, self.n_chunks, self.l2 = len(segments), int(n_chunks.value), float(l2)
        self.seg = torch.tensor([int(x) for s in segments for x in s], dtype=torch.int64).to(device)
        self.coef = torch.zeros(self.n_seg, dtype=torch.float32, device=device)
        self.reg = torch.zeros(1, dtype=torch.float32, device=device)
        self.ws = torch.zeros(self.n_chunks + 1, dtype=torch.float64, device=device)

    def launch(self, p: torch.Tensor):
        _lib.require_device()
        _chk(p, torch.float32, "p")
        call("srfrd_param_l2", _p(p), _p(self.seg), self.n_seg, self.n_chunks, self.l2, _p(self.coef), _p(self.reg),
             _p(self.ws), _stream())


def _l2_args(l2: Optional[ParamL2]):
    return (None, 0, None, None) if l2 is None else (_p(l2.seg), l2.n_seg, _p(l2.coef), _p(l2.reg))


def catalogue_topk_plan(U, n_rows, row_lo, D, n_split, k=10) -> int:
    out = C.c_int(0)
    call("srfrd_catalogue_topk_plan", U, n_rows, row_lo, D, n_split, C.byref(out), int(k))
    return out.value


def catalogue_topk_kmax(D, n_split) -> int:
    out = C.c_int(0)
    call("srfrd_catalogue_topk_kmax", D, n_split, C.byref(out))
    return out.value


def catalogue_topk(feats, U, u_pad, n_split, table, row_lo, id_base, chunks, part_scores, part_ids, packed=None, k=10):
    _lib.require_device()
    D = table.shape[1]
    call("srfrd_catalogue_topk", _p(feats), U, u_pad, n_split, _p(table), table.shape[0], row_lo, id_base, D,
         feats.stride(0), table.stride(0), chunks, _p(part_scores), _p(part_ids), _p(packed), _stream(), int(k))


def catalogue_rank(feats, U, u_pad, n_split, table, row_lo, id_base, target_rows, target_ids, rank_out,
                   target_scores=None):
    _lib.require_device()
    D = table.shape[1]
    call("srfrd_catalogue_rank", _p(feats), U, u_pad, n_split, _p(table), table.shape[0], row_lo, id_base, D,
         feats.stride(0), table.stride(0), _p(target_rows), target_rows.stride(0), _p(target_ids), _p(target_scores),
         _p(rank_out), _stream())


def merge_topk_packed(packed, U, nlists, k, out_scores, out_ids):
    _lib.require_device()
    call("srfrd_merge_topk_packed", _p(packed), U, nlists, k, _p(out_scores), _p(out_ids), _stream())


def merge_topk(scores, ids, U, nlists, k, out_scores, out_ids):
    _lib.require_device()
    call("srfrd_merge_topk", _p(scores), _p(ids), U, nlists, k, _p(out_scores), _p(out_ids), _stream())


def sample_batch(offsets, items, labels, p_fake, eligible, itemnum, B, L, policy, seed, step, out, w_pos=None):
    _lib.require_device()
    call("srfrd_sample_batch", _p(offsets), _p(items), _p(labels), _p(p_fake), _p(eligible), eligible.numel(), int(itemnum),
         B, L, int(policy), int(seed), _p(step), _p(out.get("users")), _p(out["seq"]), _p(out["rsq"]), _p(out["pos"]),
         _p(out["prs"]), _p(out["neg"]), _p(out["nrs"]), _p(w_pos), _stream())


def sample_candidates(offsets, items, users0, target, itemnum, C, seed, cand):
    _lib.require_device()
    call("srfrd_sample_candidates", _p(offsets), _p(items), _p(users0), _p(target), users0.numel(), int(itemnum), int(C),
         int(seed), _p(cand), _stream())


def candidate_rank(feats, item_table, cand, D, fake_table=None, user_label=None, logits=None, rank=None, err_flag=None):
    _lib.require_device()
    _chk(feats, torch.float32, "feats"); _chk(item_table, torch.float32, "item_table"); _chk(cand, torch.int64, "cand")
    U, Cn = cand.shape
    F = 0 if fake_table is None else fake_table.shape[1]
    call("srfrd_candidate_rank", _p(feats), feats.stride(0), _p(item_table), item_table.shape[0], int(D), _p(cand), U, Cn,
         _p(fake_table), F, _p(user_label), _p(logits), 0 if logits is None else logits.stride(0), _p(rank), _p(err_flag),
         _stream())


def add_user_term(logits, feats_tail, fake_table, label):
    _lib.require_device()
    U, I = logits.shape
    call("srfrd_add_user_term", _p(logits), logits.stride(0), U, I, _p(feats_tail), feats_tail.stride(0), _p(fake_table),
         _p(label), fake_table.shape[1], _stream())


class PackedPlan:

    def __init__(self, B: int, L: int, device):
        self.B, self.L = B, L
        self.cap = (B * (L + 1) + 127) // 128 * 128
        i32 = lambda n: torch.zeros(n, dtype=torch.int32, device=device)
        self.rows, self.cnt, self.seq_first = i32(4), i32(B), i32(B + 1)
        self.tok_row, self.row_tok = i32(B * L), i32(self.cap)
        self.row_ids = torch.zeros(self.cap, dtype=torch.int64, device=device)
        self.row_info = i32(4 * self.cap)
        self.tile_row0, self.last_row = i32(B + 130), i32(B)
        self.desc = PackDesc(_p(self.rows), _p(self.cnt), _p(self.seq_first), _p(self.tok_row), _p(self.row_tok),
                             _p(self.row_ids), _p(self.row_info), _p(self.tile_row0), _p(self.last_row), self.cap)

    def build(self, seq, keep=None):
        _lib.require_device()
        B, L = seq.shape
        assert (B, L) == (self.B, self.L)
        _chk(seq, torch.int64, "seq")
        call("srfrd_pack_plan", _p(seq), _p(keep), B, L, C.byref(self.desc), _stream())


@contextmanager
def row_limit(rows_dev):
    call("srfrd_set_row_limit", _p(rows_dev))
    try:
        yield
    finally:
        call("srfrd_set_row_limit", None)


class LiveTiles:

    def __init__(self, B: int, L: int, heads: int, device):
        nq = (L + 127) // 128
        self.B, self.L, self.heads = B, L, heads
        self.q_lo = torch.zeros(B, dtype=torch.int32, device=device)
        self.items = torch.zeros(B * heads * nq, dtype=torch.int32, device=device)
        self.n_live = torch.zeros(1, dtype=torch.int32, device=device)

    def build(self, plan: "PackedPlan"):
        _lib.require_device()
        assert (plan.B, plan.L) == (self.B, self.L)
        self.tok_row = plan.tok_row
        call("srfrd_attention_live_items", _p(plan.tok_row), self.B, self.L, self.heads, _p(self.q_lo), _p(self.items),
             _p(self.n_live), _stream())

    @contextmanager
    def active(self):
        call("srfrd_set_attention_live", _p(self.q_lo), _p(self.items), _p(self.n_live), _p(self.tok_row))
        try:
            yield
        finally:
            call("srfrd_set_attention_live", None, None, None, None)


def attention_packed_supported(L: int, H: int, heads: int) -> bool:
    return bool(_lib.load().srfrd_attention_packed_supported(int(L), int(H), int(heads)))


def embed_ln_fwd_packed(item_table, pos_table, aux_table, mode, seq, aux_ids, item_scale, ln_w, ln_b, eps, x0_bf16, q_bf16,
                        stats, plan: PackedPlan, drop_p=0.0, drop_seed=0, drop_stream=0, drop_step=None):
    _lib.require_device()
    B, L = seq.shape
    D = item_table.shape[1]
    F = aux_table.shape[1] if (aux_table is not None and mode == 1) else 0
    call("srfrd_embed_ln_fwd_packed", _p(item_table), item_table.shape[0], D, _p(pos_table), _p(aux_table),
         0 if aux_table is None else aux_table.shape[0], F, mode, _p(seq), _p(aux_ids), B, L, float(item_scale), _p(ln_w),
         _p(ln_b), float(eps), _p(x0_bf16), _p(q_bf16), _p(stats), x0_bf16.stride(0), float(drop_p), int(drop_seed),
         int(drop_stream), _p(drop_step), _p(plan.row_tok), _p(plan.rows), plan.cap, _stream())


def layernorm_fwd_rows(x, w, b, eps, y_f32, row_index, n, H):
    _lib.require_device()
    call("srfrd_layernorm_fwd_rows", _p(x), x.stride(0), _p(w), _p(b), float(eps), _p(y_f32), y_f32.stride(0), _p(row_index),
         n, H, _stream())


def attention_packed_oproj_supported(L: int, H: int, heads: int) -> int:
    return int(_lib.load().srfrd_attention_packed_oproj_supported(int(L), int(H), int(heads)))


def attention_fwd_packed(q, k, v, o, plan: PackedPlan, L, H, heads, drop_p=0.0, seed=0, stream_id=0, drop_step=None,
                         wo=None, bias=None, residual=None, r=None, y=None, ln_w=None, ln_b=None, ln_eps=0.0, ln_stats=None):
    _lib.require_device()
    st = lambda t: 0 if t is None else t.stride(0)
    call("srfrd_attention_fwd_packed", _p(q), q.stride(0), _p(k), _p(v), k.stride(0), _p(o), o.stride(0), C.byref(plan.desc),
         L, H, heads, float(drop_p), int(seed), int(stream_id), _p(drop_step), _stream(), _p(wo), st(wo), _p(bias),
         _p(residual), st(residual), _p(ln_w), _p(ln_b), float(ln_eps), _p(ln_stats), _p(r), st(r), _p(y), st(y))


def attention_bwd_packed(dout, q, k, v, dq, dk, dv, plan: PackedPlan, L, H, heads, drop_p=0.0, seed=0, stream_id=0,
                         drop_step=None, dr=None, woT=None):
    st = lambda t: 0 if t is None else t.stride(0)
    call("srfrd_attention_bwd_packed", _p(dout), st(dout), _p(q), q.stride(0), _p(k), _p(v), k.stride(0), _p(dq),
         dq.stride(0), _p(dk), _p(dv), dk.stride(0), C.byref(plan.desc), L, H, heads, float(drop_p), int(seed),
         int(stream_id), _p(drop_step), _stream(), _p(dr), st(dr), _p(woT), st(woT))


def score_loss_fused_packed(h, item_table, fake_table, pos, neg, prs, nrs, w_pos, w_neg, norm, loss_acc, dh, d_item, d_fake,
                            plan: PackedPlan):
    D = item_table.shape[1]
    F = 0 if fake_table is None else fake_table.shape[1]
    call("srfrd_score_loss_fused_packed", _p(h), h.stride(0), _p(item_table), _p(fake_table), _p(pos), _p(neg), _p(prs),
         _p(nrs), _p(w_pos), _p(w_neg), _p(norm), D, F, _p(loss_acc), _p(dh), dh.stride(0), _p(d_item), _p(d_fake),
         _p(plan.row_tok), _p(plan.rows), plan.cap, _stream())


def embed_bwd_packed(dx0, seq, aux_ids, plan: PackedPlan, D, F, mode, item_scale, d_item, d_aux, d_pos):
    B, L = seq.shape
    call("srfrd_embed_bwd_packed", _p(dx0), dx0.stride(0), _p(seq), _p(aux_ids), _p(plan.row_tok), _p(plan.rows), plan.cap,
         L, D, F, mode, float(item_scale), _p(d_item), _p(d_aux), _p(d_pos), _stream())


def dp_adam_step(grad_ptrs_dev: int, param_ptrs_dev: int, signal_ptrs_dev: int, rank, world, n, m, v, lr, beta1, beta2, eps,
                 state8, norm2, local4, l2: Optional[ParamL2] = None):
    _lib.require_device()
    call("srfrd_dp_adam_step", grad_ptrs_dev, param_ptrs_dev, signal_ptrs_dev, int(rank), int(world), int(n), _p(m), _p(v),
         float(lr), float(beta1), float(beta2), float(eps), _p(state8), _p(norm2), _p(local4), _stream(), *_l2_args(l2))


def _parts(parts):
    arr = (RepackPart * len(parts))()
    for i, (src, dst, W, mode) in enumerate(parts):
        arr[i] = RepackPart(_p(src), src.stride(0), _p(dst), dst.stride(0), int(W), int(mode))
    return arr


def unpack_rows(parts, plan: PackedPlan):
    _lib.require_device()
    arr = _parts(parts)
    call("srfrd_unpack_rows", arr, len(parts), C.byref(plan.desc), plan.B, plan.L, _stream())


def pack_rows(parts, plan: PackedPlan):
    _lib.require_device()
    arr = _parts(parts)
    call("srfrd_pack_rows", arr, len(parts), C.byref(plan.desc), plan.B, plan.L, _stream())


def mlp2_tn(A, W1, W2, mid_out, out, bias1=None, bias2=None, gate=None, relu1=False, drop1_p=0.0, drop2_p=0.0, drop1_stream=0,
            drop2_stream=0, drop_seed=0, drop_step=None, residual=None, residual_is_a=False, row_ids=None, ln_out=None,
            ln_w=None, ln_b=None, ln_stats=None, ln_eps=0.0, M=None):
    _lib.require_device()
    M = A.shape[0] if M is None else M
    N = W1.shape[0]
    ep = Mlp2Epilogue(_p(bias1), _p(bias2), _p(gate), 0 if gate is None else gate.stride(0), int(relu1), float(drop1_p),
                      float(drop2_p), int(drop1_stream), int(drop2_stream), int(drop_seed), _p(drop_step), _p(residual),
                      0 if residual is None else residual.stride(0), int(residual_is_a), _p(row_ids), _p(mid_out),
                      mid_out.stride(0), _p(out), out.stride(0), _p(ln_out), 0 if ln_out is None else ln_out.stride(0),
                      _p(ln_w), _p(ln_b), _p(ln_stats), float(ln_eps))
    call("srfrd_mlp2_tn", _p(A), A.stride(0), _p(W1), W1.stride(0), _p(W2), W2.stride(0), M, N, C.byref(ep), _stream())
```

Baseline: 9.903 million.

## Fuse LayerNorm backward into FFN and in-projection data-grad kernels

Adds a LayerNorm-backward epilogue to the mlp2 tcgen05 kernel. The FFN backward now writes dr directly, and a new in-projection mode computes the Q and KV data-grads from one concatenated dqkv against a combined weight, then applies the attention LayerNorm backward in-kernel. LayerNorm weight and bias grads are reduced per CTA in shared memory and added to global with atomics. This removes the separate gemm_tn and layernorm_bwd launches and their intermediate round trips, at the cost of more templated kernel variants, extra shared memory and per-tile reduction work in the epilogue.

```diff
diff --git a/include/srfrd_b200.h b/include/srfrd_b200.h
--- a/include/srfrd_b200.h
+++ b/include/srfrd_b200.h
@@ -8,7 +8,7 @@
 extern "C" {
 #endif
 
-#define SRFRD_ABI_VERSION 9
+#define SRFRD_ABI_VERSION 10
 #if defined(__GNUC__)
 #define SRFRD_API __attribute__((visibility("default")))
 #else
@@ -206,6 +206,8 @@
   void* mid_out; int ldm;
   void* out; int ldc;
   void* ln_out; int ld_ln; const float* ln_w; const float* ln_b; float* ln_stats; float ln_eps;
+  const void* lnb_x; int ldlx; const float* lnb_stats; const float* lnb_w; float* lnb_dw; float* lnb_db;
+  int in_k;
 } srfrd_mlp2_t;
 SRFRD_API int srfrd_mlp2_tn(const void* A_bf16, int lda, const void* W1_bf16, int ldw1, const void* W2_bf16, int ldw2, int M, int N,
                   const srfrd_mlp2_t* ep, void* stream);
diff --git a/srfrd_b200/_lib.py b/srfrd_b200/_lib.py
--- a/srfrd_b200/_lib.py
+++ b/srfrd_b200/_lib.py
@@ -25,7 +25,8 @@
     _fields_ = [("bias1", vp), ("bias2", vp), ("gate", vp), ("ldg", i32), ("relu1", i32), ("drop1_p", f32), ("drop2_p", f32),
                 ("drop1_stream", u32), ("drop2_stream", u32), ("drop_seed", u64), ("drop_step", vp), ("residual", vp), ("ldr", i32),
                 ("residual_is_a", i32), ("row_ids", vp), ("mid_out", vp), ("ldm", i32), ("out", vp), ("ldc", i32),
-                ("ln_out", vp), ("ld_ln", i32), ("ln_w", vp), ("ln_b", vp), ("ln_stats", vp), ("ln_eps", f32)]
+                ("ln_out", vp), ("ld_ln", i32), ("ln_w", vp), ("ln_b", vp), ("ln_stats", vp), ("ln_eps", f32),
+                ("lnb_x", vp), ("ldlx", i32), ("lnb_stats", vp), ("lnb_w", vp), ("lnb_dw", vp), ("lnb_db", vp), ("in_k", i32)]
 
 
 class PackDesc(C.Structure):
@@ -122,7 +123,7 @@
         fn = getattr(lib, name)
         fn.argtypes = argtypes
         fn.restype = C.c_int
-    if lib.srfrd_abi_version() != 9:
+    if lib.srfrd_abi_version() != 10:
         raise RuntimeError("srfrd_b200: ABI version mismatch between _lib.py and the built library")
     _lib = lib
     return lib
diff --git a/srfrd_b200/csrc/ffn.cu b/srfrd_b200/csrc/ffn.cu
--- a/srfrd_b200/csrc/ffn.cu
+++ b/srfrd_b200/csrc/ffn.cu
@@ -1,4 +1,6 @@
 #include <stdlib.h>
+
+#include <algorithm>
 
 #include "common.cuh"
 #include "srfrd_b200.h"
@@ -24,6 +26,8 @@
   int residual_is_a;
   const int64_t* row_ids;
   const float *ln_w, *ln_b; float* ln_stats; float ln_eps; int has_ln;
+  int lnb;
+  const bf16* lnb_x; int ldlx; const float* lnb_stats; float *lnb_dw, *lnb_db;
 };
 
 __device__ __forceinline__ uint32_t swz_chunk(int r, int j) { return (uint32_t)(r * 128 + ((j ^ (r & 7)) << 4)); }
@@ -39,6 +43,83 @@
   for (int i = 0; i < 4; ++i) { f[2 * i] = __uint_as_float(w[i] << 16); f[2 * i + 1] = __uint_as_float(w[i] & 0xffff0000u); }
 }
 
+__device__ __forceinline__ float warp_transpose_sum16(float (&v)[16], int lane) {
+#pragma unroll
+  for (int o = 8; o > 0; o >>= 1) {
+    const bool up = lane & o;
+#pragma unroll
+    for (int i = 0; i < o; ++i) {
+      const float send = up ? v[i] : v[i + o], keep = up ? v[i + o] : v[i];
+      v[i] = keep + __shfl_xor_sync(0xffffffffu, send, o);
+    }
+  }
+  return v[0] + __shfl_xor_sync(0xffffffffu, v[0], 16);
+}
+
+template <int LPR, int CH, bool ADD>
+__device__ __forceinline__ void ln_bwd_row(uint8_t* sA, const uint8_t* sAdd, const float* slw, float* sdw, float* sdb,
+                                           const MlpParams& p, int r, int lane, int64_t row, bool rok, bool keep) {
+  const float invH = 1.f / (float)p.N;
+  const float2 st = rok ? __ldg(reinterpret_cast<const float2*>(p.lnb_stats + 2 * row)) : make_float2(0.f, 0.f);
+  const float rstd = st.y, nb = -st.x * st.y;
+  const bf16* xrow = p.lnb_x + (rok ? row : 0) * p.ldlx;
+  float psg[LPR], psx[LPR];
+#pragma unroll
+  for (int s = 0; s < LPR; ++s) {
+    float sg = 0.f, sgx = 0.f;
+#pragma unroll
+    for (int ch = 0; ch < CH; ++ch) {
+      const int c = (ch * LPR + s) * 8;
+      if (c >= p.N) continue;
+      float xv[8], dv[8];
+      unpack8_bf16(__ldg(reinterpret_cast<const uint4*>(xrow + c)), xv);
+      unpack8_bf16(*reinterpret_cast<const uint4*>(sA + (c >> 6) * MBLK + swz_chunk(r, (c & 63) >> 3)), dv);
+#pragma unroll
+      for (int j = 0; j < 8; ++j) {
+        const float xh = fmaf(xv[j], rstd, nb);
+        const float g = dv[j] * slw[c + j];
+        sg += g;
+        sgx = fmaf(g, xh, sgx);
+      }
+    }
+    psg[s] = sg; psx[s] = sgx;
+  }
+#pragma unroll
+  for (int o = LPR / 2; o > 0; o >>= 1)
+#pragma unroll
+    for (int s = 0; s < o; ++s) { psg[s] = psg[s] + psg[s + o]; psx[s] = psx[s] + psx[s + o]; }
+  const float sg = psg[0] * invH, sgx = psx[0] * invH;
+  constexpr int NC = LPR * CH * 8;
+#pragma unroll
+  for (int c0 = 0; c0 < NC; c0 += 16) {
+    if (c0 >= p.N) break;
+    float tw[16], tb[16];
+#pragma unroll
+    for (int q = 0; q < 2; ++q) {
+      const int c = c0 + 8 * q;
+      uint8_t* ch = sA + (c >> 6) * MBLK + swz_chunk(r, (c & 63) >> 3);
+      float xv[8], dv[8], av[8], o[8];
+      unpack8_bf16(__ldg(reinterpret_cast<const uint4*>(xrow + c)), xv);
+      unpack8_bf16(*reinterpret_cast<const uint4*>(ch), dv);
+      if (ADD) unpack8_bf16(*reinterpret_cast<const uint4*>(sAdd + (c >> 6) * MBLK + swz_chunk(r, (c & 63) >> 3)), av);
+#pragma unroll
+      for (int j = 0; j < 8; ++j) {
+        const float xh = fmaf(xv[j], rstd, nb);
+        const float u = fmaf(-sgx, xh, fmaf(dv[j], slw[c + j], -sg));
+        o[j] = ADD ? fmaf(rstd, u, av[j]) : rstd * u;
+        tw[8 * q + j] = rok ? dv[j] * xh : 0.f;
+        tb[8 * q + j] = rok ? dv[j] : 0.f;
+      }
+      uint4 pk = make_uint4(pack_bf16x2(o[0], o[1]), pack_bf16x2(o[2], o[3]), pack_bf16x2(o[4], o[5]), pack_bf16x2(o[6], o[7]));
+      if (!keep) pk = make_uint4(0, 0, 0, 0);
+      *reinterpret_cast<uint4*>(ch) = pk;
+    }
+    const float w = warp_transpose_sum16(tw, lane), b = warp_transpose_sum16(tb, lane);
+    if (lane < 16) { atomicAdd(sdw + c0 + lane, w); atomicAdd(sdb + c0 + lane, b); }
+  }
+}
+
+template <int LNB, int LPR, int CH>
 __global__ void __launch_bounds__(MLP_THREADS, 2)
 mlp2_kernel(const __grid_constant__ CUtensorMap tmA, const __grid_constant__ CUtensorMap tmW1,
             const __grid_constant__ CUtensorMap tmW2, const __grid_constant__ CUtensorMap tmMid,
@@ -46,16 +127,18 @@
   extern __shared__ uint8_t smem_raw[];
   uint8_t* smem = reinterpret_cast<uint8_t*>((reinterpret_cast<uintptr_t>(smem_raw) + 1023) & ~uintptr_t(1023));
   const int wblk = (p.N * 128 + 1023) & ~1023;
-  const int ablk = max(p.kb, p.kbk);
+  const int ablk = max(LNB == 2 ? 2 * p.kb : p.kb, p.kbk);
   uint8_t* sW1 = smem;
   uint8_t* sW2 = sW1 + p.kbk * wblk;
   uint8_t* sA = sW2 + (p.single ? 0 : p.kb) * wblk;
   uint8_t* sM = sA + ablk * MBLK;
-  float* sb1 = reinterpret_cast<float*>(sM + p.kb * MBLK);
+  float* sb1 = reinterpret_cast<float*>(sM + (LNB == 2 ? 0 : p.kb) * MBLK);
   float* sb2 = sb1 + 128;
   float* slw = sb2 + 128;
   float* slb = slw + 128;
-  uint64_t* bars = reinterpret_cast<uint64_t*>(slb + 128);
+  float* sdw = slb + 128;
+  float* sdb = sdw + 128;
+  uint64_t* bars = reinterpret_cast<uint64_t*>(slb + (LNB ? 3 : 1) * 128);
   uint64_t *w_full = bars, *a_full = bars + 1, *a_free = bars + 2, *acc1_full = bars + 3, *mid_ready = bars + 4,
            *acc2_full = bars + 5;
   uint32_t* tmem_slot = reinterpret_cast<uint32_t*>(bars + 6);
@@ -76,8 +159,9 @@
   for (int i = threadIdx.x; i < 128; i += blockDim.x) {
     sb1[i] = (p.bias1 && i < p.N) ? __ldg(p.bias1 + i) : 0.f;
     sb2[i] = (p.bias2 && i < p.N) ? __ldg(p.bias2 + i) : 0.f;
-    slw[i] = (p.has_ln && i < p.N) ? __ldg(p.ln_w + i) : 0.f;
+    slw[i] = ((LNB || p.has_ln) && i < p.N) ? __ldg(p.ln_w + i) : 0.f;
     slb[i] = (p.has_ln && i < p.N) ? __ldg(p.ln_b + i) : 0.f;
+    if (LNB) sdw[i] = sdb[i] = 0.f;
   }
   tc_fence_before();
   __syncthreads();
@@ -107,7 +191,15 @@
       if (tile == (int)blockIdx.x) mbar_wait(w_full, 0);
       mbar_wait(a_full, ph);
       tc_fence_after();
-      if (elect_one()) {
+      if (LNB == 2) {
+        if (elect_one()) {
+          const int split = p.N / 16, ksteps = p.K / 16;
+          for (int g = 0; g < ksteps; ++g)
+            umma_bf16(g < split ? tAcc1 : tAcc2, dA + (uint64_t)((g >> 2) * (MBLK >> 4) + 2 * (g & 3)),
+                      dW1 + (uint64_t)((g >> 2) * (wblk >> 4) + 2 * (g & 3)), idesc, g != 0 && g != split);
+          umma_commit(acc2_full);
+        }
+      } else if (elect_one()) {
         for (int kb = 0; kb < p.kbk; ++kb) {
           const int ksteps = min(4, (p.K - kb * 64 + 15) / 16);
           for (int k = 0; k < ksteps; ++k)
@@ -183,6 +275,36 @@
       mbar_wait(acc2_full, ph);
       tc_fence_after();
       float ln_sum = 0.f, ln_sq = 0.f;
+      if (LNB == 2) {
+#pragma unroll
+        for (int c = 0; c < LPR * CH * 8; c += 16) {
+          if (c >= p.N) break;
+          uint32_t raw1[16], raw2[16];
+          tmem_ld16(tAcc1 + lane_off + c, raw1);
+          tmem_ld16(tAcc2 + lane_off + c, raw2);
+          uint4 r0 = make_uint4(0, 0, 0, 0), r1 = r0;
+          if (rok) {
+            const uint4* rp = reinterpret_cast<const uint4*>(p.residual + row * p.ldr + c);
+            r0 = __ldg(rp); r1 = __ldg(rp + 1);
+          }
+          tmem_ld_wait();
+          float v[16], a[16], rv[16];
+          unpack8_bf16(r0, rv); unpack8_bf16(r1, rv + 8);
+#pragma unroll
+          for (int i = 0; i < 16; ++i) { v[i] = __uint_as_float(raw1[i]) + rv[i]; a[i] = __uint_as_float(raw2[i]); }
+          const int j = (c & 63) >> 3;
+          uint8_t* blk = sA + (c >> 6) * MBLK;
+          uint8_t* ablk2 = sA + (p.kb + (c >> 6)) * MBLK;
+          *reinterpret_cast<uint4*>(blk + swz_chunk(r, j)) =
+              make_uint4(pack_bf16x2(v[0], v[1]), pack_bf16x2(v[2], v[3]), pack_bf16x2(v[4], v[5]), pack_bf16x2(v[6], v[7]));
+          *reinterpret_cast<uint4*>(blk + swz_chunk(r, j + 1)) =
+              make_uint4(pack_bf16x2(v[8], v[9]), pack_bf16x2(v[10], v[11]), pack_bf16x2(v[12], v[13]), pack_bf16x2(v[14], v[15]));
+          *reinterpret_cast<uint4*>(ablk2 + swz_chunk(r, j)) =
+              make_uint4(pack_bf16x2(a[0], a[1]), pack_bf16x2(a[2], a[3]), pack_bf16x2(a[4], a[5]), pack_bf16x2(a[6], a[7]));
+          *reinterpret_cast<uint4*>(ablk2 + swz_chunk(r, j + 1)) =
+              make_uint4(pack_bf16x2(a[8], a[9]), pack_bf16x2(a[10], a[11]), pack_bf16x2(a[12], a[13]), pack_bf16x2(a[14], a[15]));
+        }
+      } else
 #pragma unroll 1
       for (int c = 0; c < p.N; c += 16) {
         uint32_t raw[16];
@@ -214,7 +336,7 @@
           if (p.relu2) x = fmaxf(x, 0.f);
           if (p.gate2) x = gv2[i] > 0.f ? x : 0.f;
           x += rv[i];
-          v[i] = x * rowm;
+          v[i] = LNB ? x : x * rowm;
         }
         const uint4 p0 = make_uint4(pack_bf16x2(v[0], v[1]), pack_bf16x2(v[2], v[3]), pack_bf16x2(v[4], v[5]), pack_bf16x2(v[6], v[7]));
         const uint4 p1 = make_uint4(pack_bf16x2(v[8], v[9]), pack_bf16x2(v[10], v[11]), pack_bf16x2(v[12], v[13]), pack_bf16x2(v[14], v[15]));
@@ -228,7 +350,8 @@
         }
       }
       tc_fence_before();
-      if (p.has_ln) {
+      if (LNB) ln_bwd_row<LPR, CH, LNB == 2>(sA, sA + p.kb * MBLK, slw, sdw, sdb, p, r, lane, row, rok, rowm != 0.f);
+      if (!LNB && p.has_ln) {
         if (issuer) asm volatile("cp.async.bulk.wait_group.read 0;" ::: "memory");
         mlp_bar_sync();
         const float invn = 1.f / (float)p.N;
@@ -260,6 +383,10 @@
       }
     }
     if (issuer) asm volatile("cp.async.bulk.wait_group 0;" ::: "memory");
+    if (LNB && (int)blockIdx.x < n_tiles) {
+      mlp_bar_sync();
+      for (int i = threadIdx.x; i < p.N; i += 128) { red_add_f32(p.lnb_dw + i, sdw[i]); red_add_f32(p.lnb_db + i, sdb[i]); }
+    }
   }
   tc_fence_before();
   __syncthreads();
@@ -269,6 +396,30 @@
 }
 
 using namespace srfrd;
+
+template <int LNB, int LPR, int CH>
+static int mlp_launch_k(const MlpParams& p, size_t smem, int64_t grid, cudaStream_t stream, const CUtensorMap& tmA,
+                        const CUtensorMap& tmW1, const CUtensorMap& tmW2, const CUtensorMap& tmMid, const CUtensorMap& tmOut,
+                        const CUtensorMap& tmLn) {
+  static bool attr = false;
+  if (!attr) {
+    SRFRD_CUDA(cudaFuncSetAttribute(mlp2_kernel<LNB, LPR, CH>, cudaFuncAttributeMaxDynamicSharedMemorySize, 200 * 1024));
+    attr = true;
+  }
+  SRFRD_CUDA(launch_pdl(mlp2_kernel<LNB, LPR, CH>, dim3((unsigned)grid), dim3(MLP_THREADS), smem, stream, tmA, tmW1, tmW2, tmMid,
+                        tmOut, tmLn, p));
+  return 0;
+}
+
+template <int LNB>
+static int mlp_launch_lnb(const MlpParams& p, size_t smem, int64_t grid, cudaStream_t stream, const CUtensorMap& tmA,
+                          const CUtensorMap& tmW1, const CUtensorMap& tmW2, const CUtensorMap& tmMid, const CUtensorMap& tmOut,
+                          const CUtensorMap& tmLn) {
+  if (p.N <= 32) return mlp_launch_k<LNB, 4, 1>(p, smem, grid, stream, tmA, tmW1, tmW2, tmMid, tmOut, tmLn);
+  if (p.N <= 64) return mlp_launch_k<LNB, 8, 1>(p, smem, grid, stream, tmA, tmW1, tmW2, tmMid, tmOut, tmLn);
+  if (p.N <= 96) return mlp_launch_k<LNB, 4, 3>(p, smem, grid, stream, tmA, tmW1, tmW2, tmMid, tmOut, tmLn);
+  return mlp_launch_k<LNB, 16, 1>(p, smem, grid, stream, tmA, tmW1, tmW2, tmMid, tmOut, tmLn);
+}
 
 static int mlp_launch(MlpParams& p, const void* A, int lda, const void* W1, int ldw1, const void* W2, int ldw2, void* mid_out,
                       int ldm, void* out, int ldc, void* ln_out, int ld_ln, cudaStream_t stream) {
@@ -286,17 +437,17 @@
   tmLn = tmOut;
   if (p.has_ln) if (int rc = make_tmap_bf16_2d(&tmLn, ln_out, p.M, p.N, ld_ln, MT, 64)) return rc;
   const int wblk = (p.N * 128 + 1023) & ~1023;
-  const int ablk = p.kb > p.kbk ? p.kb : p.kbk;
-  const size_t smem = 1024 + (size_t)(p.kbk + (p.single ? 0 : p.kb)) * wblk + (size_t)(ablk + p.kb) * MBLK + 4 * 128 * sizeof(float) + 128;
-  static bool attr = false;
-  if (!attr) {
-    SRFRD_CUDA(cudaFuncSetAttribute(mlp2_kernel, cudaFuncAttributeMaxDynamicSharedMemorySize, 200 * 1024));
-    attr = true;
-  }
+  const int ablk = std::max(p.lnb == 2 ? 2 * p.kb : p.kb, p.kbk);
+  const int mblk = p.lnb == 2 ? 0 : p.kb;
+  const size_t smem = 1024 + (size_t)(p.kbk + (p.single ? 0 : p.kb)) * wblk + (size_t)(ablk + mblk) * MBLK +
+                      (p.lnb ? 6 : 4) * 128 * sizeof(float) + 128;
   SRFRD_REQUIRE(smem <= 200 * 1024, "mlp2_tn: shared memory %zu too large", smem);
   int64_t grid = ((int64_t)p.M + MT - 1) / MT;
   if (grid > 2 * num_sms()) grid = 2 * num_sms();
-  SRFRD_CUDA(launch_pdl(mlp2_kernel, dim3((unsigned)grid), dim3(MLP_THREADS), smem, stream, tmA, tmW1, tmW2, tmMid, tmOut, tmLn, p));
+  int rc = p.lnb == 1 ? mlp_launch_lnb<1>(p, smem, grid, stream, tmA, tmW1, tmW2, tmMid, tmOut, tmLn)
+         : p.lnb == 2 ? mlp_launch_lnb<2>(p, smem, grid, stream, tmA, tmW1, tmW2, tmMid, tmOut, tmLn)
+                      : mlp_launch_k<0, 1, 1>(p, smem, grid, stream, tmA, tmW1, tmW2, tmMid, tmOut, tmLn);
+  if (rc) return rc;
   SRFRD_LAUNCH_CHECK();
   return 0;
 }
@@ -332,16 +483,27 @@
 extern "C" int srfrd_mlp2_tn(const void* A, int lda, const void* W1, int ldw1, const void* W2, int ldw2, int M, int N,
                              const srfrd_mlp2_t* ep, void* stream_) {
   cudaStream_t stream = (cudaStream_t)stream_;
-  SRFRD_REQUIRE(A && W1 && W2 && ep && ep->mid_out && ep->out, "mlp2_tn: null pointer");
+  SRFRD_REQUIRE(A && W1 && ep && ep->out, "mlp2_tn: null pointer");
   SRFRD_REQUIRE(M > 0 && N >= 16 && N <= 128 && N % 16 == 0, "mlp2_tn: N = K must be a multiple of 16 up to 128 (got %d)", N);
-  SRFRD_REQUIRE(lda % 8 == 0 && ldw1 % 8 == 0 && ldw2 % 8 == 0 && ep->ldm % 8 == 0 && ep->ldc % 8 == 0 && lda >= N && ldw1 >= N &&
-                    ldw2 >= N && ep->ldm >= N && ep->ldc >= N, "mlp2_tn: bad leading dimensions");
+  const int in = ep->in_k != 0;
+  const int K = in ? 3 * N : N;
+  SRFRD_REQUIRE(!in || ep->in_k == 3 * N, "mlp2_tn: in_k must be 3 N (got %d, N = %d)", ep->in_k, N);
+  SRFRD_REQUIRE(in || (W2 && ep->mid_out), "mlp2_tn: null pointer");
+  SRFRD_REQUIRE(lda % 8 == 0 && ldw1 % 8 == 0 && ep->ldc % 8 == 0 && lda >= K && ldw1 >= K && ep->ldc >= N &&
+                    (in || (ldw2 % 8 == 0 && ep->ldm % 8 == 0 && ldw2 >= N && ep->ldm >= N)), "mlp2_tn: bad leading dimensions");
   SRFRD_REQUIRE(!ep->gate || (ep->ldg % 8 == 0 && ((uintptr_t)ep->gate & 15) == 0), "mlp2_tn: bad gate");
   SRFRD_REQUIRE(!ep->residual || (ep->ldr % 8 == 0 && ((uintptr_t)ep->residual & 15) == 0), "mlp2_tn: bad residual");
   SRFRD_REQUIRE(!ep->ln_out || (ep->ln_w && ep->ln_b && ep->ld_ln % 8 == 0 && ep->ld_ln >= N), "mlp2_tn: bad LayerNorm arguments");
   SRFRD_REQUIRE(ep->drop1_p >= 0.f && ep->drop1_p < 1.f && ep->drop2_p >= 0.f && ep->drop2_p < 1.f, "mlp2_tn: dropout p must be in [0, 1)");
+  const int lnb = ep->lnb_x ? 1 + in : 0;
+  SRFRD_REQUIRE(!in || lnb, "mlp2_tn: the in-projection mode needs the LayerNorm backward");
+  SRFRD_REQUIRE(!lnb || (ep->lnb_stats && ep->lnb_w && ep->lnb_dw && ep->lnb_db && ep->ldlx % 8 == 0 && ep->ldlx >= N &&
+                         ((uintptr_t)ep->lnb_x & 15) == 0 && !ep->ln_out && !ep->bias2 && ep->drop2_p == 0.f),
+                "mlp2_tn: bad LayerNorm-backward arguments (no ln_out, bias2 or drop2 with it)");
+  SRFRD_REQUIRE(!in || (ep->residual && !ep->residual_is_a && !ep->gate && !ep->bias1 && ep->drop1_p == 0.f && !ep->relu1),
+                "mlp2_tn: the in-projection mode takes a residual and no first-stage epilogue");
   MlpParams p = {};
-  p.M = M; p.N = N; p.K = N; p.single = 0;
+  p.M = M; p.N = N; p.K = K; p.single = in;
   p.bias1 = ep->bias1; p.bias2 = ep->bias2; p.gate = (const bf16*)ep->gate; p.ldg = ep->ldg; p.relu1 = ep->relu1;
   p.drop_seed = ep->drop_seed; p.drop_step = ep->drop_step; p.stream1 = ep->drop1_stream; p.stream2 = ep->drop2_stream;
   p.thresh1 = ep->drop1_p > 0.f ? (uint32_t)((double)ep->drop1_p * 4294967296.0) : 0;
@@ -349,9 +511,12 @@
   p.scale1 = ep->drop1_p > 0.f ? 1.f / (1.f - ep->drop1_p) : 1.f;
   p.scale2 = ep->drop2_p > 0.f ? 1.f / (1.f - ep->drop2_p) : 1.f;
   p.residual = (const bf16*)ep->residual; p.ldr = ep->ldr;
-  p.residual_is_a = (ep->residual == nullptr && ep->residual_is_a) || (ep->residual == A && ep->ldr == lda);
+  p.residual_is_a = !in && ((ep->residual == nullptr && ep->residual_is_a) || (ep->residual == A && ep->ldr == lda));
   if (p.residual_is_a) p.residual = nullptr;
   p.row_ids = ep->row_ids;
-  p.ln_w = ep->ln_w; p.ln_b = ep->ln_b; p.ln_stats = ep->ln_stats; p.ln_eps = ep->ln_eps;
-  return mlp_launch(p, A, lda, W1, ldw1, W2, ldw2, ep->mid_out, ep->ldm, ep->out, ep->ldc, ep->ln_out, ep->ld_ln, stream);
-}
+  p.ln_w = lnb ? ep->lnb_w : ep->ln_w; p.ln_b = ep->ln_b; p.ln_stats = ep->ln_stats; p.ln_eps = ep->ln_eps;
+  p.lnb = lnb; p.lnb_x = (const bf16*)ep->lnb_x; p.ldlx = ep->ldlx; p.lnb_stats = ep->lnb_stats;
+  p.lnb_dw = ep->lnb_dw; p.lnb_db = ep->lnb_db;
+  return mlp_launch(p, A, lda, W1, ldw1, in ? W1 : W2, in ? ldw1 : ldw2, ep->mid_out, ep->ldm, ep->out, ep->ldc, ep->ln_out,
+                    ep->ld_ln, stream);
+}
diff --git a/srfrd_b200/engine.py b/srfrd_b200/engine.py
--- a/srfrd_b200/engine.py
+++ b/srfrd_b200/engine.py
@@ -186,8 +186,9 @@
             bin_ = P.view(f"attention_layers.{i}.in_proj_bias")
             self.sh[f"wq{i}"] = zb(Hp, Hp)
             self.sh[f"wkv{i}"] = zb(2 * Hp, Hp)
-            self.sh[f"wqT{i}"] = zb(Hp, Hp)
-            self.sh[f"wkvT{i}"] = zb(Hp, 2 * Hp)
+            self.sh[f"winT{i}"] = zb(Hp, 3 * Hp)
+            self.sh[f"wqT{i}"] = self.sh[f"winT{i}"][:, :Hp]
+            self.sh[f"wkvT{i}"] = self.sh[f"winT{i}"][:, Hp:]
             entries.append((win[:H], self.sh[f"wq{i}"][:H, :H], self.sh[f"wqT{i}"][:H, :H]))
             entries.append((win[H:2 * H], self.sh[f"wkv{i}"][:H, :H], self.sh[f"wkvT{i}"][:H, :H]))
             entries.append((win[2 * H:], self.sh[f"wkv{i}"][Hp:Hp + H, :H], self.sh[f"wkvT{i}"][:H, Hp:Hp + H]))
@@ -269,10 +270,10 @@
         for n in ("gA", "gC", "gD", "gX"):
             act(n)
         for i in range(nb):
-            for n in ("gda1_", "gdr_", "gdq_"):
+            for n in ("gda1_", "gdr_"):
                 act(f"{n}{i}")
             act(f"gdz_{i}")
-            act(f"gdkv_{i}", 2 * H)
+            act(f"gdqkv_{i}", 3 * H)
         if s.kind == "SRFR":
             act("gc", s.Dp)
         if s.dropout > 0:
@@ -445,7 +446,8 @@
 
         for i in reversed(range(nb)):
             Q, q, kv, o, r, y, h1 = (ws[f"{n}{i}"][:T] for n in ("Q", "q", "kv", "o", "r", "y", "h1"))
-            dz, da1, dr, dq, dkv = (ws[f"{n}{i}"][:T] for n in ("gdz_", "gda1_", "gdr_", "gdq_", "gdkv_"))
+            dz, da1, dr, dqkv = (ws[f"{n}{i}"][:T] for n in ("gdz_", "gda1_", "gdr_", "gdqkv_"))
+            dq, dkv = dqkv[:, :Hp], dqkv[:, Hp:]
             dx_out = ws[f"gdz_{i - 1}"][:T] if i > 0 else gA
             dz2 = dz
             if p_drop > 0:
@@ -619,7 +621,9 @@
         GM = lambda name: P.mat(name, grad=True)
         x = [ws[f"x{i}"][:T] for i in range(nb + 1)]
         dz_top = ws[f"gdz_{nb - 1}"][:T]
-        fuse_oproj = self._fuse_oproj(hyb, L, Hp <= 128 and os.environ.get("SRFRD_FUSE_LN", "1") != "0") & 2
+        fuse_ln = Hp <= 128 and os.environ.get("SRFRD_FUSE_LN", "1") != "0"
+        fuse_oproj = self._fuse_oproj(hyb, L, fuse_ln) & 2
+        fuse_lnb = fuse_ln and hyb is None
         with ops.row_limit(plan.rows):
             if s.kind == "SRFR":
                 gc = ws["gc"][:T]
@@ -633,7 +637,8 @@
                                   G("last_layernorm.weight"), G("last_layernorm.bias"), row_ids=row_ids, H=s.Dout)
             for i in reversed(range(nb)):
                 Q, q, kv, o, r, y, h1 = (ws[f"{n}{i}"][:T] for n in ("Q", "q", "kv", "o", "r", "y", "h1"))
-                dz, da1, dr, dq, dkv = (ws[f"{n}{i}"][:T] for n in ("gdz_", "gda1_", "gdr_", "gdq_", "gdkv_"))
+                dz, da1, dr, dqkv = (ws[f"{n}{i}"][:T] for n in ("gdz_", "gda1_", "gdr_", "gdqkv_"))
+                dq, dkv = dqkv[:, :Hp], dqkv[:, Hp:]
                 dx_out = ws[f"gdz_{i - 1}"][:T] if i > 0 else gA
                 dz2 = dz
                 if p_drop > 0:
@@ -641,9 +646,13 @@
                     ops.dropout_apply(dz, dz2, Hp, p_drop, seed, 12 + 4 * i, step)
                 with self._branch():
                     ops.gemm_wgrad(dz2, h1, GM(f"forward_layers.{i}.conv2.weight"), G(f"forward_layers.{i}.conv2.bias"), Mo=H, No=H)
+                ln2 = (P.view(f"forward_layernorms.{i}.weight"), G(f"forward_layernorms.{i}.weight"),
+                       G(f"forward_layernorms.{i}.bias"))
+                ln2_fused = fuse_lnb and self.fuse_ffn
                 if self.fuse_ffn and Hp <= 128:
-                    ops.mlp2_tn(dz2, self.sh[f"w2T{i}"], self.sh[f"w1T{i}"], da1, gC, gate=h1, drop1_p=p_drop,
-                                drop1_stream=11 + 4 * i, drop_seed=seed, drop_step=step, residual=dz)
+                    lnb = dict(lnb_x=r, lnb_stats=ws[f"st2_{i}"][:T], lnb_w=ln2[0], lnb_dw=ln2[1], lnb_db=ln2[2]) if ln2_fused else {}
+                    ops.mlp2_tn(dz2, self.sh[f"w2T{i}"], self.sh[f"w1T{i}"], da1, dr if ln2_fused else gC, gate=h1,
+                                drop1_p=p_drop, drop1_stream=11 + 4 * i, drop_seed=seed, drop_step=step, residual=dz, **lnb)
                     with self._branch():
                         ops.gemm_wgrad(da1, y, GM(f"forward_layers.{i}.conv1.weight"), G(f"forward_layers.{i}.conv1.bias"),
                                        Mo=H, No=H)
@@ -654,8 +663,8 @@
                         ops.gemm_wgrad(da1, y, GM(f"forward_layers.{i}.conv1.weight"), G(f"forward_layers.{i}.conv1.bias"),
                                        Mo=H, No=H)
                     ops.gemm_tn(da1, self.sh[f"w1T{i}"], out_bf16=gC, residual=dz)
-                ops.layernorm_bwd(gC, r, ws[f"st2_{i}"][:T], P.view(f"forward_layernorms.{i}.weight"), dr,
-                                  G(f"forward_layernorms.{i}.weight"), G(f"forward_layernorms.{i}.bias"), H=H)
+                if not ln2_fused:
+                    ops.layernorm_bwd(gC, r, ws[f"st2_{i}"][:T], ln2[0], dr, ln2[1], ln2[2], H=H)
                 with self._branch():
                     ops.gemm_wgrad(dr, o, GM(f"attention_layers.{i}.out_proj.weight"),
                                    G(f"attention_layers.{i}.out_proj.bias"), Mo=H, No=H)
@@ -681,13 +690,17 @@
                 with self._branch():
                     ops.gemm_wgrad(dq, Q, gin[:H], gbin[:H], Mo=H, No=H)
                     ops.gemm_wgrad(dkv, x[i], gin[H:], gbin[H:], Mo=2 * H, No=H)
-                with self._branch(second=True):
-                    ops.gemm_tn(dkv, self.sh[f"wkvT{i}"], out_bf16=gX)
-                ops.gemm_tn(dq, self.sh[f"wqT{i}"], out_bf16=gD, residual=dr)
-                self._join(second=True)
-                ops.layernorm_bwd(gD, x[i], ws[f"st1_{i}"][:T], P.view(f"attention_layernorms.{i}.weight"), dx_out,
-                                  G(f"attention_layernorms.{i}.weight"), G(f"attention_layernorms.{i}.bias"),
-                                  add=gX, row_ids=row_ids, H=H)
+                ln1 = (P.view(f"attention_layernorms.{i}.weight"), G(f"attention_layernorms.{i}.weight"),
+                       G(f"attention_layernorms.{i}.bias"))
+                if fuse_lnb:
+                    ops.mlp2_tn(dqkv, self.sh[f"winT{i}"], None, None, dx_out, residual=dr, row_ids=row_ids, lnb_x=x[i],
+                                lnb_stats=ws[f"st1_{i}"][:T], lnb_w=ln1[0], lnb_dw=ln1[1], lnb_db=ln1[2], in_proj=True)
+                else:
+                    with self._branch(second=True):
+                        ops.gemm_tn(dkv, self.sh[f"wkvT{i}"], out_bf16=gX)
+                    ops.gemm_tn(dq, self.sh[f"wqT{i}"], out_bf16=gD, residual=dr)
+                    self._join(second=True)
+                    ops.layernorm_bwd(gD, x[i], ws[f"st1_{i}"][:T], ln1[0], dx_out, ln1[1], ln1[2], add=gX, row_ids=row_ids, H=H)
             dx0 = gA
             if s.kind == "SASRec" and p_drop > 0:
                 ops.dropout_apply(gA, gC, H, p_drop, seed, 1, step)
diff --git a/srfrd_b200/ops.py b/srfrd_b200/ops.py
--- a/srfrd_b200/ops.py
+++ b/srfrd_b200/ops.py
@@ -444,13 +444,19 @@
 
 def mlp2_tn(A, W1, W2, mid_out, out, bias1=None, bias2=None, gate=None, relu1=False, drop1_p=0.0, drop2_p=0.0, drop1_stream=0,
             drop2_stream=0, drop_seed=0, drop_step=None, residual=None, residual_is_a=False, row_ids=None, ln_out=None,
-            ln_w=None, ln_b=None, ln_stats=None, ln_eps=0.0, M=None):
+            ln_w=None, ln_b=None, ln_stats=None, ln_eps=0.0, lnb_x=None, lnb_stats=None, lnb_w=None, lnb_dw=None,
+            lnb_db=None, in_proj=False, M=None):
     _lib.require_device()
     M = A.shape[0] if M is None else M
     N = W1.shape[0]
+    if in_proj:
+        W2 = mid_out = None
     ep = Mlp2Epilogue(_p(bias1), _p(bias2), _p(gate), 0 if gate is None else gate.stride(0), int(relu1), float(drop1_p),
                       float(drop2_p), int(drop1_stream), int(drop2_stream), int(drop_seed), _p(drop_step), _p(residual),
                       0 if residual is None else residual.stride(0), int(residual_is_a), _p(row_ids), _p(mid_out),
-                      mid_out.stride(0), _p(out), out.stride(0), _p(ln_out), 0 if ln_out is None else ln_out.stride(0),
-                      _p(ln_w), _p(ln_b), _p(ln_stats), float(ln_eps))
-    call("srfrd_mlp2_tn", _p(A), A.stride(0), _p(W1), W1.stride(0), _p(W2), W2.stride(0), M, N, C.byref(ep), _stream())
+                      0 if mid_out is None else mid_out.stride(0), _p(out), out.stride(0), _p(ln_out),
+                      0 if ln_out is None else ln_out.stride(0), _p(ln_w), _p(ln_b), _p(ln_stats), float(ln_eps), _p(lnb_x),
+                      0 if lnb_x is None else lnb_x.stride(0), _p(lnb_stats), _p(lnb_w), _p(lnb_dw), _p(lnb_db),
+                      3 * N if in_proj else 0)
+    call("srfrd_mlp2_tn", _p(A), A.stride(0), _p(W1), W1.stride(0), _p(W2), 0 if W2 is None else W2.stride(0), M, N,
+         C.byref(ep), _stream())
```

Result: no change. 9.919 million (median of 6 runs) (+0.2%).
